# kieranrcampbell/clonealign

Hardware: AMD Instinct MI355X
Metric: ELBO iterations/sec (higher is better)
Workload: dtype f32 variables (contraction: float64 series over gene bins; count-matrix products: int8 MFMA, exact); 1 GPU; synthetic 100000 cells x 5000 genes x 8 clones, K=1, S=1, cell-sharded over 1 GPU(s) (BASELINE.json configs[2]); cells=100000, genes=5000, clones=8, K=1, mc_samples=1, y_storage=u8, y_bytes_per_elem=1, fused_sweep=True, fwd_mfma=True, series_form=True, y_mfma=True, parallelism=single, collective=none, allreduce_doubles_per_train_pass=20764, build_id=212aa564458010f1

## Files before the change

clonealign_amd/csrc/ca_eng_create.inc:

```

constexpr double CA_ML_STREAM_FIXED_US = 6.6;
constexpr double CA_ML_STREAM_BYTES_PER_US = 5.62e6;
constexpr double CA_ML_MIN_STREAM_US = 45.0;
constexpr int CA_ML_MAX_PER = 4;
struct ca_mom_last_in {
  int slots;
  int n_cu;
  int nb_stream, nb_ovf;
  int ngrp, nred;
  int64_t image_bytes;
};
inline int ca_mom_last_free(const ca_mom_last_in& a) { return std::max(a.slots - a.nb_stream, 0); }
inline int ca_mom_last_free_x(const ca_mom_last_in& a) {
  const int xcd = std::max(a.n_cu / 32, 1);
  return a.slots / xcd - cdiv(a.nb_stream, xcd);
}
inline int ca_mom_last_per(const ca_mom_last_in& a) {
  const int xcd = std::max(a.n_cu / 32, 1), free_x = ca_mom_last_free_x(a);
  if (free_x < 1) return 0;
  return std::max(1, cdiv(a.ngrp, free_x * xcd));
}
inline bool ca_mom_last_pick(const ca_mom_last_in& a) {
  if (a.nb_stream + a.ngrp + a.nred <= a.slots) return false;
  const int per = ca_mom_last_per(a);
// ... 413 lines not shown
          HIPCK(h, hipGetLastError());
          int total = 0;
          HIPCK(h, hipMemcpyAsync(&total, h->esc2_off + nkeys, sizeof(int), hipMemcpyDeviceToHost, h->stream));
          SYNC(h);
          if ((int64_t)total != ne) { h->err = "2-bit image: the device's escape count differs from the host plan's"; return CA_ERR_STATE; }
          h->n_esc2 = total;
          CACK(dalloc(h, &h->esc2, h->n_esc2));
          hipLaunchKernelGGL(k_esc_fill, dim3(cdiv(nw * 64, CA_YM_TB)), dim3(CA_YM_TB), 0, h->stream, (const uint8_t*)h->Y, Nn, h->Gp, h->ys_nseg, h->ys_RS,
                             h->esc2_off, h->esc2, (const uint4*)h->y2_pos, n2);
          const int64_t sb = n2 * 1024 + (8 - n2) * 2048, ib = (h->ys_N64 / 64) * h->ys_nseg * sb;
          CACK(dalloc(h, &h->Ys2, ib));
          hipLaunchKernelGGL(k_pack_y2, dim3(cdiv(ib / 16, CA_YM_TB)), dim3(CA_YM_TB), 0, h->stream, (const uint8_t*)h->Y, (uint4*)h->Ys2, Nn, h->ys_N64, h->Gp, n2,
                             h->y2_perm);
          HIPCK(h, hipGetLastError());
          SYNC(h);
          h->ys_n2 = n2;
          h->y_dev_bytes += ib + 4 * h->n_esc2 + 4 * (nkeys + 1) + 4 * (int64_t)h->Gp;
        }
      }
    }
    if (h->adam_bound > 0) h->ys_step_bound = (float)(1.02 * h->adam_bound);
    h->y_ys = true;
    h->y_dev_bytes += h->ys4 ? h->ys_N64 * h->Gp / 2 + 4 * h->n_esc + 4 * ((int64_t)h->ys_nrg * h->ys_nseg * 4 * h->ys_RS + 1) : h->ys_N64 * h->Gp;
  }
  h->mom_ride = h->poly && h->y_ys && !h->poly_side && h->host_dev && variant_on(h, CA_VAR_MOM_RIDE, "CA_MOM_RIDE");
  if (h->mom_ride) {
    ca_mom_last_in ml;
    int per_cu = 0;
    const hipError_t oe = h->ys4 ? (h->n_ovf > 0 ? hipOccupancyMaxActiveBlocksPerMultiprocessor(&per_cu, k_ys_mfma_ovf_mom<true>, CA_YM_TB, CA_YS4_LDS_BYTES)
                                                 : hipOccupancyMaxActiveBlocksPerMultiprocessor(&per_cu, k_ys_mfma_mom<true>, CA_YM_TB, CA_YS4_LDS_BYTES))
                                 : (h->n_ovf > 0 ? hipOccupancyMaxActiveBlocksPerMultiprocessor(&per_cu, k_ys_mfma_ovf_mom<false>, CA_YM_TB, CA_YS_LDS_BYTES)
                                                 : hipOccupancyMaxActiveBlocksPerMultiprocessor(&per_cu, k_ys_mfma_mom<false>, CA_YM_TB, CA_YS_LDS_BYTES));
    if (oe != hipSuccess) { (void)hipGetLastError(); per_cu = 0; }
    ml.slots = per_cu * h->n_cu; ml.n_cu = h->n_cu;
    ml.nb_stream = h->ys_nrg * h->ys_nseg;
    ml.nb_ovf = h->n_ovf > 0 ? cdiv(Nn, CA_TB) + cdiv(h->n_ovf_chunk, CA_TB / 64) : 0;
    ml.ngrp = h->pws.n_gene_blocks; ml.nred = CA_MOM_NRED;
    ml.image_bytes = h->ys_N64 * h->Gp / (h->ys4 ? 2 : 1);
    h->mom_free_slots = ca_mom_last_free(ml);
    h->mom_last = variantx_on(h, CA_VARX_MOM_LAST, "CA_MOM_LAST_ON") || (variant_on(h, CA_VAR_MOM_LAST, "CA_MOM_LAST") && ca_mom_last_pick(ml));
    if (h->opt.variant_off & CA_VAR_MOM_LAST) h->mom_last = false;
    if (h->mom_last) {
      const int per = ca_mom_last_per(ml);
      h->mom_per = per < 1 ? CA_MOM_PER : std::min(per, CA_ML_MAX_PER);
      h->mom_nred = 2 * CA_MOM_NRED;
      const int lab = (h->opt.reserved[1] & ~0xFF) ? h->opt.reserved[1] >> 8 : 0;
      if (lab & 15) h->mom_per = lab & 15;
      if (lab & 16) h->mom_nred = CA_MOM_NRED;
      h->mom_ovf_first = (lab & 32) != 0;
    }
  }
  h->cell_lean = h->poly && variant_on(h, CA_VAR_CELL_LEAN, "CA_CELL_LEAN");
  h->cell_mfma = h->poly && variant_on(h, CA_VAR_CELL_MFMA, "CA_CELL_MFMA");
  h->ride_ok = h->ystore == CA_YSTORE_U8 && K == 1 && D <= 2 && h->fused_ok && !h->c16 && h->fwd_cell && (h->fc_tl == 6 || h->fc_tl == 8 || (h->fc_tl == 2 && h->fc_nbig == 0)) &&
               !h->y_ys && variant_on(h, CA_VAR_Y_RIDE, "CA_Y_RIDE");
  const bool tl1_ok = h->fc_tl == 1 && h->fc_nbig == 0 && !h->c16;
  h->ride_ys = h->y_ys && (!h->ys4 || (h->poly && D == 1 && !h->c16 && !h->s2)) && D <= 2 && h->fused_ok && h->fwd_cell && (h->fc_tl == 6 || tl1_ok || (h->fc_tl == 2 && h->fc_nbig == 0)) &&
               variant_on(h, CA_VAR_Y_RIDE, "CA_Y_RIDE");
  h->yfin_split = h->ride_ys && h->bwd_mfma && h->tail_fuse && variant_on(h, CA_VAR_YFIN_RIDE, "CA_YFIN_RIDE");
  if (h->y_ys && !h->ride_ys) h->async_y = false;
  {
    const int tiles = cdiv(Nn, 16), qb = tiles / std::max(h->n_cu, 1), rb = tiles - qb * h->n_cu;
    h->fwd_bal = h->ride_ys && !h->c16 && !h->s2 && D == 1 && C <= 8 && qb >= 1 && qb <= 6 && h->nk32 >= 96 && h->host_dev && variant_on(h, CA_VAR_FWD_BAL, "CA_FWD_BAL");
    if (h->fwd_bal) {
      h->bal_q = qb; h->bal_r = rb;
      h->bal_nchunk = rb > 0 ? std::min(CA_BAL_MAXCHUNK, h->n_cu / rb) : 0;
      CACK(dalloc(h, &h->bal_xw, std::max<int64_t>(1, (int64_t)rb * h->bal_nchunk * 512)));
    }
  }
  h->s2f = h->s2 && h->fused_ok && h->fwd_cell && (h->fc_tl == 2 || h->fc_tl == 6) && (h->ride_ys || !h->ride_ok) && variant_on(h, CA_VAR_S2_FUSE, "CA_S2_FUSE");
  h->layout_series = h->poly || (h->poly_shape && h->opt.world > 1);
  if (h->layout_series) {
    h->off_y = 3 + C;
    h->off_q = h->off_y + (int64_t)h->Gp * K;
    h->off_x = h->off_q + (int64_t)CA_PL_NB * (CA_PL_R + 2) * 8;
    h->off_g = h->off_x + std::max(h->opt.world, 1);
    h->red_n = h->off_g + (int64_t)G * (S + D);
    CACK(dalloc(h, &h->red, h->red_n));
    if (h->poly) h->pws.tabQ = h->red + h->off_q;
  } else {
  h->off_g = 3 + C;
  h->off_y = h->off_g + (int64_t)G * (S + D);
  h->red_n = h->off_y + (int64_t)G * K;
  CACK(dalloc(h, &h->red, h->off_y + (int64_t)h->Gp * std::max(K, 1)));
  }
  CACK(dalloc(h, &h->terms_dev, 4));
  CACK(ensure_elbo_cap(h, 64));
  CACK(ensure_eps_cap(h, 1));
  {
    const int cols = 1 + ((K > 0) ? P : 0);
    const int cols_all = cols + (p->loc0 ? 0 : 1);
    std::vector<double> srow;
    if (!p->loc0) {
      srow.resize((size_t)Nn);
      HIPCK(h, hipMemcpyAsync(srow.data(), h->s64, (size_t)Nn * sizeof(double), hipMemcpyDeviceToHost, h->stream));
      SYNC(h);
    }
    std::vector<double> cs((size_t)G, 0.0), ytx((size_t)G * std::max(P, 1), 0.0);
    float *Ft = nullptr, *Vt = nullptr, *YWp = nullptr, *YTp = nullptr; double* yt = nullptr;
    HIPCK(h, hipMalloc((void**)&Ft, (size_t)Nn * sizeof(float)));
    HIPCK(h, hipMalloc((void**)&Vt, (size_t)G * sizeof(float)));
    HIPCK(h, hipMalloc((void**)&YWp, (size_t)h->nseg * Nn * sizeof(float)));
    HIPCK(h, hipMalloc((void**)&YTp, (size_t)h->nrb * h->Gp * sizeof(float)));
    HIPCK(h, hipMalloc((void**)&yt, (size_t)h->Gp * sizeof(double)));
    HIPCK(h, hipMemsetAsync(Vt, 0, (size_t)G * sizeof(float), h->stream));
    std::vector<float> col((size_t)Nn);
// ... 63 lines not shown
```

clonealign_amd/csrc/ca_eng_loop.inc:

```
int wait_y(ca_engine* h, bool all) {
  if (all) {
    if (h->y_pending) HIPCK(h, hipStreamWaitEvent(h->stream, h->ev_ydone, 0));
    h->y_pending = false; h->yw_pending = false;
  } else if (h->yw_pending) {
    HIPCK(h, hipStreamWaitEvent(h->stream, h->ev_ywdone, 0));
    h->yw_pending = false;
  }
  return CA_OK;
}

int make_etamax(ca_engine* h) {
  if (h->D > 0) {
    LAUNCH(h, CA_KERNEL_OTHER, hipLaunchKernelGGL(k_vmm_final, dim3(1), dim3(64), 0, h->stream, h->vmm_part, h->vmm, h->ngblk, h->D));
    LAUNCH(h, CA_KERNEL_OTHER, hipLaunchKernelGGL(k_etamax, dim3(cdiv(h->N, CA_TB)), dim3(CA_TB), 0, h->stream, h->F, h->vmm, h->etamax2, h->N, h->D));
  }
  h->em_stale = false;
  return CA_OK;
}
int ensure_etamax(ca_engine* h) {
  if (!h->em_stale) return CA_OK;
  return make_etamax(h);
}

int refresh_derived(ca_engine* h) {
  CACK(wait_y(h, true));
  h->y_defer = false;
  h->pre_valid = false;
  h->ys_steps = -1;
  h->ys_quant_ready = false;
  if (h->D > 0) LAUNCH(h, CA_KERNEL_OTHER, hipLaunchKernelGGL(k_vprep, dim3(h->ngblk), dim3(CA_TB), 0, h->stream, h->V, h->Vs, h->vmm_part, h->G, h->D));
  CACK(make_etamax(h));
  h->gaux_slot = -1;
  h->ycache_valid = false;
  h->yfin_pending = false;
  h->look_valid = false;
  h->poly_fresh = false;
  h->poly_seq_base = h->poly_seq + 1;
  h->poly_xmax_ready = false;
  h->poly_xglob_steps = -1;
  return CA_OK;
}

ca_ovf_args ovf_args(ca_engine* h, float* YWextra) {
  ca_ovf_args ovf;
  memset(&ovf, 0, sizeof(ovf));
  if (h->n_ovf > 0) {
    ovf.nb_rows = cdiv(h->N, CA_TB); ovf.nb_chunks = cdiv(h->n_ovf_chunk, CA_TB / 64);
    ovf.rowptr = h->ovf_rowptr; ovf.col = h->ovf_col; ovf.val = h->ovf_val; ovf.YWextra = YWextra;
    ovf.chunk_start = h->ovf_chunk_start; ovf.row2 = h->ovf_row2; ovf.val2 = h->ovf_val2; ovf.csum = h->ovf_csum; ovf.nchunk = h->n_ovf_chunk;
  }
  return ovf;
}
ca_yfin_args yfin_args(ca_engine* h, int rows, int nseg) {
  ca_yfin_args a;
  memset(&a, 0, sizeof(a));
  a.ncol = cdiv((int64_t)h->Gp * h->K, 64); a.nrow = h->n_yw;
  a.part = h->YTpart; a.out = h->red + h->off_y; a.rows = rows; a.ld = (int64_t)h->Gp * h->K; a.cols = h->Gp * h->K; a.G = h->G;
  if (h->n_ovf > 0) { a.col_chunk_ptr = h->ovf_col_chunk_ptr; a.csum = h->ovf_csum; }
  a.YWpart = h->YWpart; a.nseg = nseg + (h->n_ovf > 0 ? 1 : 0); a.F = h->F; a.D = h->D; a.N = h->N; a.YW = h->YW; a.yw_part = h->yw_part;
  return a;
}
int launch_yfinish(ca_engine* h, int rows, int nseg) {
  const ca_yfin_args a = yfin_args(h, rows, nseg);
  LAUNCH(h, CA_KERNEL_OTHER, hipLaunchKernelGGL(k_yfinish, dim3(a.ncol + a.nrow), dim3(1024), 0, h->stream, a.part, a.out, a.rows, a.ld, a.cols, a.col_chunk_ptr,
                                                a.csum, h->K, a.G, a.ncol, a.YWpart, a.nseg, a.F, a.D, a.N, a.YW, a.yw_part));
  return CA_OK;
}

ca_ysq_args ys_quant_args(ca_engine* h, int steps, bool* lagged) {
  ca_ysq_args a;
  memset(&a, 0, sizeof(a));
  const int s0 = h->ys_slot, s1 = (s0 + 1) % 3;
  a.nblk = h->ys_nq;
  a.V = h->V; a.Dv = h->D; a.G = h->G; a.GS = h->Gp / 64; a.F = h->F; a.Df = h->D; a.N = h->N; a.NS = h->ys_N64 / 64;
  *lagged = steps >= 0 && steps <= 4 && h->ys_step_bound > 0.f;
  if (*lagged) {
    a.amax_in = h->ys_amaxp + (int64_t)s0 * h->ys_ncap * 2; a.n_in = h->ys_namax[s0];
    a.slack_w = a.slack_p = (float)steps * h->ys_step_bound;
  } else {
    a.amax_in = reinterpret_cast<const float*>(h->ys_amax); a.n_in = 1;
  }
  a.amax_out = h->ys_amaxp + (int64_t)s1 * h->ys_ncap * 2;
  h->ys_namax[s1] = h->ys_nq;
  a.exps = h->ys_exps + 2 * s0; a.Wr = h->Wr; a.Pr = h->Pr; a.Wsum = h->Wsum; a.Psum = h->Psum;
  return a;
}
int ys_quant(ca_engine* h) {
  if (h->ys_quant_ready) return CA_OK;
  bool lagged = false;
  ca_ysq_args a = ys_quant_args(h, h->ys_steps, &lagged);
  if (!lagged) {
    HIPCK(h, hipMemsetAsync(h->ys_amax, 0, 2 * sizeof(unsigned), h->stream));
    LAUNCH(h, CA_KERNEL_OTHER, hipLaunchKernelGGL(k_ym_absmax, dim3(cdiv(std::max<int64_t>(h->N, h->G), CA_YM_TB)), dim3(CA_YM_TB), 0, h->stream,
                                                  h->V, h->D, (int64_t)h->G, h->F, h->D, h->N, 1, h->ys_amax));
  }
  LAUNCH(h, CA_KERNEL_OTHER, hipLaunchKernelGGL(k_ys_quant, dim3(a.nblk), dim3(CA_YM_TB), 0, h->stream, a));
  return CA_OK;
}
ca_ys_io ys_io(ca_engine* h) {
  ca_ys_io io;
  io.Wr = h->Wr; io.Pr = h->Pr; io.Wsum = h->Wsum; io.Psum = h->Psum; io.exps = h->ys_exps + 2 * h->ys_slot;
  io.YWpart = h->YWpart; io.YTpart = h->YTpart;
  io.esc_off = h->ys4 ? h->esc_off : nullptr; io.esc = h->ys4 ? h->esc : nullptr;
  io.perm = nullptr;
  return io;
}
ca_ovf_args ys_ovf(ca_engine* h) { return ovf_args(h, h->YWpart + (int64_t)h->ys_nseg * h->N); }
int yfin_flush(ca_engine* h) {
  if (!h->yfin_pending) return CA_OK;
  h->yfin_pending = false;
  return launch_yfinish(h, h->ys_nrg, h->ys_nseg);
}
int ys_finish(ca_engine* h, bool defer = false) {
  h->yfin_pending = true;
  if (!defer) CACK(yfin_flush(h));
  h->ys_slot = (h->ys_slot + 1) % 3;
  h->ys_launched = true;
  h->ys_steps = 0;
  h->ys_quant_ready = false;
  h->ycache_valid = true;
  return CA_OK;
}
template <bool Y4, int N2 = 0>
void launch_ys(ca_engine* h) {
  constexpr int lds = Y4 ? CA_YS4_LDS_BYTES : CA_YS_LDS_BYTES;
  ca_ys_io yio = ys_io(h);
  const uint8_t* Yimg = h->Ys;
  if (N2 > 0) { Yimg = h->Ys2; yio.esc_off = h->esc2_off; yio.esc = h->esc2; yio.perm = h->y2_perm; }
  const int nb_main = h->ys_nrg * h->ys_nseg;
  const ca_pm_args* pm = h->mom_args;
  h->mom_args = nullptr;
  const int nmom = pm ? pm->nmb + pm->nred : 0;
  if (h->n_ovf > 0) {
    const ca_ovf_args ovf = ys_ovf(h);
    const dim3 grid(nmom + nb_main + ovf.nb_rows + ovf.nb_chunks);
    if (pm) {
      ca_pm_args pmo = *pm;
      if (h->mom_last && h->mom_ovf_first) pmo.blk0 += ovf.nb_rows + ovf.nb_chunks;
      hipLaunchKernelGGL((k_ys_mfma_ovf_mom<Y4, N2>), grid, dim3(CA_YM_TB), lds, h->stream, Yimg, yio, h->N, h->Gp, h->ys_RS, nb_main, ovf, h->F, h->V, h->D, pmo);
    }
    else hipLaunchKernelGGL((k_ys_mfma_ovf<Y4, N2>), grid, dim3(CA_YM_TB), lds, h->stream, Yimg, yio, h->N, h->Gp, h->ys_RS, nb_main, ovf, h->F, h->V, h->D);
  } else {
    if (pm) hipLaunchKernelGGL((k_ys_mfma_mom<Y4, N2>), dim3(nmom + nb_main), dim3(CA_YM_TB), lds, h->stream, Yimg, yio, h->N, h->Gp, h->ys_RS, *pm);
    else hipLaunchKernelGGL((k_ys_mfma<Y4, N2>), dim3(nb_main), dim3(CA_YM_TB), lds, h->stream, Yimg, yio, h->N, h->Gp, h->ys_RS);
  }
}
int ycache_ys(ca_engine* h) {
  CACK(ys_quant(h));
  if (h->ys4 && h->ys_n2 == 6) LAUNCH(h, CA_KERNEL_YPASS, (launch_ys<true, 6>(h)));
  else if (h->ys4 && h->ys_n2 == 5) LAUNCH(h, CA_KERNEL_YPASS, (launch_ys<true, 5>(h)));
  else if (h->ys4) LAUNCH(h, CA_KERNEL_YPASS, launch_ys<true>(h));
  else LAUNCH(h, CA_KERNEL_YPASS, launch_ys<false>(h));
  const bool defer = h->ys_defer_next;
  h->ys_defer_next = false;
  return ys_finish(h, defer);
}

int ensure_ycache(ca_engine* h) {
  if (h->y_defer) {
    h->y_defer = false;
    HIPCK(h, hipStreamWaitEvent(h->stream2, h->ev_params, 0));
    std::swap(h->stream, h->stream2);
    h->on_side = true;
    const int rc = ensure_ycache(h);
    h->on_side = false;
    std::swap(h->stream, h->stream2);
    CACK(rc);
    HIPCK(h, hipEventRecord(h->ev_ydone, h->stream2));
    h->y_pending = true;
    HIPCK(h, hipEventRecord(h->ev_ywdone, h->stream2));
    h->yw_pending = true;
    return CA_OK;
  }
  if (h->ycache_valid || h->K == 0) { h->ycache_valid = true; return yfin_flush(h); }
  h->yfin_pending = false;
  if (h->y_ys) return ycache_ys(h);
  dim3 grid((unsigned)((int64_t)h->nrg * h->nseg));
  const ca_ovf_args ovf = ovf_args(h, h->YWpart + (int64_t)h->nseg * h->N * h->K);
  ca_ovf_args none;
  memset(&none, 0, sizeof(none));
  const ca_ypass_ops fit = {h->F, h->D, h->V, h->YWpart, h->YTpart, h->K};
  for (int koff = 0; koff < h->K; koff += 4) {
    const int kk = std::min(4, h->K - koff);
    CACK(prof_begin(h, CA_KERNEL_YPASS));
    const ca_ovf_args& o = koff == 0 ? ovf : none;
    ypass<0>(h, fit, koff, kk, grid, o);
    HIPCK(h, hipGetLastError());
    CACK(prof_end(h));
  }
  if (!h->on_side) {
    CACK(launch_yfinish(h, h->nrg, h->nseg));
  } else {
    LAUNCH(h, CA_KERNEL_OTHER, hipLaunchKernelGGL(k_colsum, dim3(cdiv((int64_t)h->Gp * h->K, 64)), dim3(1024), 0, h->stream,
                                                  h->YTpart, h->red + h->off_y, h->nrg, (int64_t)h->Gp * h->K, h->Gp * h->K,
                                                  h->n_ovf > 0 ? h->ovf_col_chunk_ptr : nullptr, h->n_ovf > 0 ? h->ovf_csum : nullptr, h->K, h->G));
    LAUNCH(h, CA_KERNEL_OTHER, hipLaunchKernelGGL(k_yw_dot, dim3(h->n_yw), dim3(CA_TB), 0, h->stream, h->YWpart,
                                                  h->nseg + (h->n_ovf > 0 ? 1 : 0), h->F, h->D, h->K, h->N, h->YW, h->yw_part));
  }
  h->ycache_valid = true;
  return CA_OK;
}


ca_small_args small_args(ca_engine* h, const double* gene_part, int apply, float lr_t, double* elbo_dst, bool reduce_cells) {
  ca_small_args a;
  a.enabled = 1;
  a.red = h->red; a.gene_part = gene_part; a.ngblk = h->ngblk;
  a.vchi = h->vchi; a.alpha_u = h->alpha_u; a.m_v = h->m_v; a.v_v = h->v_v; a.m_a = h->m_a; a.v_a = h->v_a; a.g_v = h->g_v; a.g_a = h->g_a;
  a.elbo_out = elbo_dst; a.terms_out = h->terms_dev;
  a.G = h->G; a.C = h->C; a.K = h->K; a.apply = apply;
  a.lr_t = lr_t; a.b1 = (float)h->opt.beta1; a.b2 = (float)h->opt.beta2; a.aeps = (float)h->opt.adam_eps;
  a.vmm_part = h->vmm_part; a.vmm = h->vmm; a.D = h->D;
  a.dir_const = h->dir_const;
  a.cell_part = reduce_cells ? h->cell_part : nullptr; a.ncblk = h->ncblk;
  a.host_out = nullptr; a.host_flag = nullptr; a.host_seq = 0; a.reduce_only = 0;
  a.yw_part = nullptr; a.n_yw = 0;
  a.ee_part = nullptr; a.n_ee = 0;
  a.vchi_out = nullptr; a.alpha_out = nullptr;
  if (!apply && elbo_dst && h->host_seq_next && h->host_dev) {
    a.host_out = h->host_dev + 32;
    a.host_flag = reinterpret_cast<unsigned long long*>(h->host_dev + 33);
    a.host_seq = h->host_seq_next;
    h->host_seq_next = 0;
  }
  return a;
}
int mon_tail_local_sums(ca_engine* h) {
  if (!h->mon_tail.enabled || !h->mon_tail.cell_part) return CA_OK;
  CACK(wait_y(h, false));
  ca_small_args r = h->mon_tail;
  r.reduce_only = 1; r.host_out = nullptr;
  LAUNCH(h, CA_KERNEL_OTHER, hipLaunchKernelGGL(k_final_small, dim3(1), dim3(CA_TB), 0, h->stream, r));
  h->mon_tail.cell_part = nullptr; h->mon_tail.yw_part = nullptr;
  return CA_OK;
}
int flush_mon_tail(ca_engine* h) {
  if (!h->mon_tail.enabled) return CA_OK;
  CACK(wait_y(h, false));
  if (h->mon_tail.yw_part) CACK(yfin_flush(h));
  if (is_sharded(h) && (h->mon_tail.cell_part || h->mon_tail_local)) {
    CACK(mon_tail_local_sums(h));
    CACK(allreduce(h, h->red, 3 + h->C));
    h->mon_tail_local = false;
  }
  LAUNCH(h, CA_KERNEL_OTHER, hipLaunchKernelGGL(k_final_small, dim3(1), dim3(CA_TB), 0, h->stream, h->mon_tail));
  h->mon_tail.enabled = 0;
  return CA_OK;
}

#ifndef CA_BWD_TL3_MAXN
#define CA_BWD_TL3_MAXN 18432
#endif
int train_bwd(ca_engine* h, const float* mu32, bool cell_sums_global) {
  const int W_ = h->S + h->D;
  bool merged = false, ride_ar = false;
  ca_ar_ride ride;
  if (h->poly_fresh) {
    h->poly_fresh = false;
    h->fold_now = false;
    CACK(yfin_flush(h));
    ca_small_args bwd_tail = no_small_args();
    if (is_sharded(h)) {
      bool local_sums = false;
      if (h->mon_tail.enabled && h->mon_tail.cell_part) { CACK(mon_tail_local_sums(h)); local_sums = true; }
      else if (h->mon_tail.enabled && h->mon_tail_local) local_sums = true;
      h->mon_tail_local = false;
      CACK(wait_y(h, true));
      if (!h->poly_xslot_pending)
        HIPCK(h, ca_poly_xslot(h->stream, h->poly_xmax_ready ? h->poly_xpart : nullptr, (int)cdiv(h->N, CA_TB), h->F, h->N, h->red + h->off_x, h->opt.rank,
                               std::max(h->opt.world, 1)));
      h->poly_xslot_pending = false;
      const int64_t skip = (cell_sums_global && !local_sums) ? 3 + h->C : 0;
      CACK(allreduce(h, h->red + skip, h->off_g - skip));
      h->poly_xglob_steps = 0;
      CACK(prof_begin(h, CA_KERNEL_BWD));
      const hipError_t e = ca_poly_backward(h->stream, &h->pws, h->V, mu32, h->Lb, h->G, h->C, h->red + h->off_g, nullptr);
      HIPCK(h, e);
      CACK(prof_end(h));
      h->poly_df = true;
      h->ycache_valid = false;
      return CA_OK;
    }
    else if (h->mon_tail.enabled && h->mon_tail.cell_part && h->upd_merge && h->opt.reserved[1] != 6) {
      CACK(wait_y(h, false));
      bwd_tail = h->mon_tail;
      bwd_tail.reduce_only = 1; bwd_tail.host_out = nullptr;
      h->mon_tail.cell_part = nullptr; h->mon_tail.yw_part = nullptr;
    }
    else if (h->mon_tail.enabled) { CACK(wait_y(h, false)); bwd_tail = h->mon_tail; h->mon_tail.enabled = 0; }
    CACK(prof_begin(h, CA_KERNEL_BWD));
    const hipError_t e = ca_poly_backward(h->stream, &h->pws, h->V, mu32, h->Lb, h->G, h->C, h->red + h->off_g, &bwd_tail);
    HIPCK(h, e);
    CACK(prof_end(h));
    h->poly_df = true;
  } else
  if (h->bwd_mfma) {
    h->poly_df = false;
    const int xb = cdiv(h->nwt, CA_TB / 64);
    ca_yfin_args yfin;
    memset(&yfin, 0, sizeof(yfin));
    ride_ar = is_sharded(h) && p2p_ride_ok(h, h->red_n);
    if (is_sharded(h) && !ride_ar) CACK(yfin_flush(h));
    if (h->yfin_pending) { yfin = yfin_args(h, h->ys_nrg, h->ys_nseg); h->yfin_pending = false; }
    ca_small_args bwd_tail = no_small_args();
    bool split_tail = false;
    if (h->mon_tail.enabled && h->mon_tail.cell_part) {
      CACK(wait_y(h, false));
      bwd_tail = h->mon_tail;
      merged = is_sharded(h);
      if (merged) { bwd_tail.reduce_only = 1; bwd_tail.host_out = nullptr; }
      if (merged && ride_ar && yfin.nrow > 0 && bwd_tail.yw_part) {
        ride.yw_part = bwd_tail.yw_part; ride.n_yw = bwd_tail.n_yw; ride.yw_index = 0;
        bwd_tail.yw_part = nullptr;
      }
      split_tail = !merged && yfin.nrow > 0 && bwd_tail.yw_part != nullptr;
      if (split_tail) { bwd_tail.reduce_only = 1; bwd_tail.host_out = nullptr; bwd_tail.yw_part = nullptr; }
    }
    const int nextra = (bwd_tail.enabled || yfin.nrow) ? 1 + cdiv(yfin.ncol, CA_TB / 64) + yfin.nrow : 0;
    const ca_bwdm_extra extra = {bwd_tail, yfin, cdiv(nextra, xb)};
    const bool s2b = h->s2f && h->S == 2 && !h->c16;
    ca_bwdm_ops o;
    memset(&o, 0, sizeof(o));
    if (h->bwd_pairs) {
      for (int s = 0; s < h->S; ++s)
        for (int pr = 0; pr < h->bwd_pairs; ++pr) {
          const bool lone = (h->nchunk & 1) && pr == h->bwd_pairs - 1;
          o.coefq = h->coefq + ((int64_t)s * h->bwd_pairs + pr) * h->N16 * 32; o.Lb = h->Lb + (int64_t)pr * 2 * h->G * CA_CW; o.mu = mu32 + (int64_t)s * h->G;
          o.sidx = s; o.first_s = pr == 0 ? 1 : 0; o.extra = (s == 0 && pr == 0) ? &extra : nullptr;
          o.c16 = !lone;
          o.coefq1 = lone ? nullptr : h->coefq + ((int64_t)(h->S + s) * h->bwd_pairs + pr) * h->N16 * 32;
          CACK(launch_bwd_mfma(h, h->D == 1 ? 1 : 2, o));
        }
    } else {
      o.Lb = h->Lb; o.first_s = 1; o.frac = h->bwd_frac; o.c16 = h->c16; o.s2 = s2b; o.tl3 = h->bwd_tl == 3;
      if ((h->D == 1 || h->D == 2) && (s2b || h->c16)) o.coefq1 = h->coefq + h->N16 * 32;
      if ((h->D == 1 || h->D == 2) && s2b) o.mu1 = mu32 + h->G;
      for (int s = 0; s < (s2b ? 1 : h->S); ++s) {
        o.coefq = h->coefq + (int64_t)s * h->N16 * 32; o.mu = mu32 + (int64_t)s * h->G; o.sidx = s; o.extra = s == 0 ? &extra : nullptr;
        CACK(launch_bwd_mfma(h, h->D, o));
      }
    }
    if (bwd_tail.enabled) {
      if (merged) { h->mon_tail.cell_part = nullptr; h->mon_tail.yw_part = nullptr; }
      else if (split_tail) h->mon_tail.cell_part = nullptr;
      else h->mon_tail.enabled = 0;
    }
    h->fold_now = h->fold_gsum && !is_sharded(h);
    if (ride_ar) { ride.gpart = h->gpart; ride.nslice = h->csplit_m; ride.fold_n = (int64_t)h->G * W_; }
    else if (!h->fold_now)
      LAUNCH(h, CA_KERNEL_OTHER,
             hipLaunchKernelGGL(k_colsum, dim3(cdiv((int64_t)h->G * W_, 64)), dim3(1024), 0, h->stream, h->gpart,
                                h->red + h->off_g, h->csplit_m, (int64_t)h->G * W_, h->G * W_));
  } else {
    h->fold_now = false;
// ... 20 lines not shown
  CACK(wait_y(h, true));
  if (h->poly && is_sharded(h)) {
    HIPCK(h, ca_poly_xslot(h->stream, h->poly_xmax_ready ? h->poly_xpart : nullptr, (int)cdiv(h->N, CA_TB), h->F, h->N, h->red + h->off_x, h->opt.rank,
                           std::max(h->opt.world, 1)));
    h->poly_xglob_steps = 0;
    h->poly_xslot_pending = false;
  }
  const int64_t skip = (cell_sums_global && !merged) ? 3 + h->C : 0;
  ride.fold_lo = h->off_g - skip;
  CACK(allreduce(h, h->red + skip, h->red_n - skip, ride_ar ? &ride : nullptr));
  if (is_sharded(h)) h->ycache_valid = false;
  return CA_OK;
}

inline bool update_merges(const ca_engine* h, int apply, const double* elbo_dst) {
  const int64_t mB = h->s2 ? 2 * h->hint_A + 1 : h->hint_B;
  return apply && h->upd_merge && !elbo_dst && h->pre_ok && h->hint_A >= 0 && mB >= 0 && h->fused_ok && h->gene_part_alt && h->fwd_cell && h->K > 0;
}
ca_pre_args pre_args(const ca_engine* h, int64_t A, int64_t B) {
  ca_pre_args pre;
  memset(&pre, 0, sizeof(pre));
  pre.nblk = h->ngblk;
  pre.loc = h->loc; pre.ls = h->ls; pre.epsA = h->eps_dev + A * (int64_t)h->G; pre.epsB = h->eps_dev + B * (int64_t)h->G;
  pre.colsum = h->colsum; pre.Lb = h->Lb; pre.V = h->V; pre.YtX = h->YtX; pre.muA = h->mu32; pre.muB = h->s2 ? h->mu32 + h->G : h->mu32B; pre.Mb = h->Mb2;
  pre.s2 = h->s2 ? 1 : 0;
  pre.gene_partA = h->gene_part_alt; pre.gene_partB = h->gene_partB_alt; pre.Mq = h->fwd_mfma ? h->Mq : nullptr;
  pre.G = h->G; pre.D = h->D; pre.K = h->K; pre.mrow = h->frow; pre.C = h->C;
  return pre;
}
ca_ysq_args ys_quant_ride(ca_engine* h) {
  ca_ysq_args a;
  memset(&a, 0, sizeof(a));
  if (!h->y_ys || h->K == 0 || h->ys_quant_ready) return a;
  bool lagged = false;
  const ca_ysq_args q = ys_quant_args(h, h->ys_steps >= 0 ? h->ys_steps + 1 : -1, &lagged);
  if (!lagged) return a;
  h->ys_quant_ready = true;
  return q;
}
int defer_y_to_side(ca_engine* h) {
  if (!h->async_y || h->K == 0 || h->ride_ok || h->ride_ys) return CA_OK;
  HIPCK(h, hipEventRecord(h->ev_params, h->stream));
  h->y_defer = true;
  return CA_OK;
}
void adam_stepped(ca_engine* h, bool xmax_ready) {
  if (h->ys_steps >= 0) h->ys_steps += 1;
  h->b1p *= (float)h->opt.beta1;
  h->b2p *= (float)h->opt.beta2;
  h->adam_steps += 1;
  h->poly_xmax_ready = xmax_ready;
  if (h->poly_xglob_steps >= 0) h->poly_xglob_steps += 1;
  h->ycache_valid = false;
  h->yfin_pending = false;
  h->look_valid = false;
  if (h->poly && h->y_ys && h->K > 0) h->poly_y_defer = true;
}
int train_update(ca_engine* h, const float* eps, int apply, double* elbo_dst) {
  const int N256 = cdiv(h->N, CA_TB);
  float lr_t = 0.f;
  if (apply) {
    lr_t = (float)h->opt.learning_rate * sqrtf(1.f - h->b2p) / (1.f - h->b1p);
  }
  CACK(yfin_flush(h));
  ca_small_args mon = no_small_args();
  if (h->mon_tail.enabled) { mon = h->mon_tail; h->mon_tail.enabled = 0; }
  ca_psi_args psi;
  memset(&psi, 0, sizeof(psi));
  if (h->K > 0) {
    psi.nblk = N256; psi.F = h->F; psi.YW = h->YW; psi.dFpart = h->dFpart; psi.m_psi = h->m_psi; psi.v_psi = h->v_psi; psi.g_psi = h->g_psi;
    psi.N = h->N; psi.D = h->D; psi.K = h->K; psi.ntile = h->poly_df ? 1 : h->bwd_mfma ? cdiv(h->nwt, CA_TB / 64) : h->ntile;
  }
  h->pre_valid = false;
  {
    int64_t mA = h->hint_A, mB = h->hint_B;
    if (h->s2) { mA = 2 * h->hint_A; mB = mA + 1; }
    if (update_merges(h, apply, elbo_dst)) {
      ca_merge_args mg;
      memset(&mg, 0, sizeof(mg));
      h->gate_armed = false;
      if (h->gate_req && h->host_dev) {
        mg.gate = reinterpret_cast<const unsigned long long*>(h->host_dev + 48); mg.gate_seq = ++h->gate_seq;
        mg.gate_ack = reinterpret_cast<unsigned long long*>(h->host_dev + 56);
        mg.gate_err = reinterpret_cast<unsigned long long*>(h->host_dev + 40);
        mg.gate_local = h->gate_local;
        mg.gate_timeout = h->gate_ticks;
        h->gate_armed = true;
        h->gate_t0 = std::chrono::steady_clock::now();
      }
      h->gate_req = false;
      mg.pre = pre_args(h, mA, mB);
      mg.ysq = ys_quant_ride(h);
      if (mg.ysq.nblk) {
        mg.ysq.nblk = h->ngblk + N256;
        h->ys_namax[(h->ys_slot + 1) % 3] = h->ngblk + N256;
      }
      mg.tail = small_args(h, h->gene_part, 1, lr_t, nullptr, false);
      mg.tail.terms_out = nullptr;
      mg.tail.vmm_part = nullptr; mg.tail.vmm = nullptr;
      mg.tail.vchi_out = h->vchi_alt; mg.tail.alpha_out = h->alpha_u_alt;
      mg.glogit = h->glogit; mg.dgl = h->dgl; mg.m_gl = h->m_gl; mg.v_gl = h->v_gl; mg.C = h->C; mg.ncell = N256;
      if (!h->vmm_at_ready) {
        int init[32];
        for (int i = 0; i < 32; ++i) init[i] = (i & 8) ? (int)0x807FFFFF  : (int)0x7F800000 ;
        HIPCK(h, hipMemcpyAsync(h->vmm_at, init, sizeof(init), hipMemcpyHostToDevice, h->stream));
        HIPCK(h, hipStreamSynchronize(h->stream));
        h->vmm_at_ready = true;
// ... 116 lines not shown
      const hipError_t q = hipStreamQuery(h->stream);
      if (q != hipSuccess && q != hipErrorNotReady) HIPCK(h, q);
      if ((q == hipSuccess && e[0] != (double)want) || std::chrono::steady_clock::now() >= t_end) {
        h->err = "internal: the ranges of an earlier pass never reached the host (series form's look ahead)";
        return CA_ERR_STATE;
      }
    }
  }
  std::atomic_thread_fence(std::memory_order_acquire);
  out[0] = e[1]; out[1] = e[2]; out[2] = e[3];
  return CA_OK;
}
struct ca_xsrc { const float* xpart; int nx; const double* xglob; int nglob; double xadd; };
inline double poly_step_bound(const ca_engine* h) {
  return h->adam_bound * 1.0001;
}
int poly_xsrc(ca_engine* h, ca_xsrc* x) {
  memset(x, 0, sizeof(*x));
  const int nx = (int)cdiv(h->N, CA_TB);
  if (is_sharded(h)) {
    const int W = std::max(h->opt.world, 1);
    if (h->poly_xglob_steps < 0 || h->poly_xglob_steps > 1) {
      HIPCK(h, ca_poly_xslot(h->stream, h->poly_xmax_ready ? h->poly_xpart : nullptr, nx, h->F, h->N, h->red + h->off_x, h->opt.rank, W));
      CACK(allreduce(h, h->red + h->off_x, W));
      h->poly_xglob_steps = 0;
      h->poly_xslot_pending = false;
    }
    x->xglob = h->red + h->off_x; x->nglob = W; x->xadd = (double)h->poly_xglob_steps * poly_step_bound(h);
  } else if (h->poly_xmax_ready) { x->xpart = h->poly_xpart; x->nx = nx; }
  return CA_OK;
}
int poly_guard(ca_engine* h, bool* use_series, double** mirror, double* seq, bool* ranges_queued) {
  const uint64_t s = h->poly_seq + 1;
  *ranges_queued = false;
  *mirror = h->poly_ring_dev + (s % 16) * 4;
  *seq = (double)s;
  double r[3];
  int steps;
  if (s < h->poly_seq_base + CA_POLY_LAG) {
    if (s == h->poly_seq_base) {
      ca_xsrc xs;
      CACK(poly_xsrc(h, &xs));
      HIPCK(h, ca_poly_ranges(h->stream, &h->pws, h->V, h->F, h->G, h->N, *mirror, *seq, xs.xpart, xs.nx, xs.xglob, xs.nglob, xs.xadd));
      *ranges_queued = true;
      h->poly_steps_at[s % 16] = h->adam_steps;
    }
    CACK(poly_wait_entry(h, h->poly_seq_base, r));
    steps = (int)(h->adam_steps - h->poly_steps_at[h->poly_seq_base % 16]);
  } else {
    CACK(poly_wait_entry(h, s - CA_POLY_LAG, r));
    steps = (int)(h->adam_steps - h->poly_steps_at[(s - CA_POLY_LAG) % 16]);
  }
  *use_series = ca_poly_covers(r[0], r[1], r[2], steps, poly_step_bound(h));
  h->poly_seq = s;
  h->poly_steps_at[s % 16] = h->adam_steps;
  return CA_OK;
}

int fused_pass(ca_engine* h, int64_t slotA, int64_t slotB, double* elbo_dst, double* elbo_dstB = nullptr, int64_t trainA = -1) {
  const bool s2f = trainA >= 0;
  const float* epsA = h->eps_dev + slotA * (int64_t)h->G;
  const float* epsB = h->eps_dev + slotB * (int64_t)h->G;
  if (elbo_dstB) CACK(flush_mon_tail(h));
  if (h->pre_valid && h->pre_A == slotA && h->pre_B == slotB) {
    std::swap(h->gene_part, h->gene_part_alt);
    std::swap(h->gene_partB, h->gene_partB_alt);
  } else {
    LAUNCH(h, CA_KERNEL_OTHER,
           hipLaunchKernelGGL(k_gene_pre_fused, dim3(h->ngblk), dim3(CA_TB), 0, h->stream, h->loc, h->ls, epsA, epsB, h->colsum, h->Lb,
                              h->V, h->D, h->K, h->YtX, h->mu32, h->s2 ? h->mu32 + h->G : h->mu32B, h->Mb2, h->gene_part, h->gene_partB, h->G,
                              h->frow, h->C, h->fwd_mfma ? h->Mq : nullptr, h->s2 ? 1 : 0));
  }
  if (s2f) {
    const float* epsTA = h->eps_dev + trainA * (int64_t)h->G;
    LAUNCH(h, CA_KERNEL_OTHER,
           hipLaunchKernelGGL(k_gene_pre_fused, dim3(h->ngblk), dim3(CA_TB), 0, h->stream, h->loc, h->ls, epsTA, epsTA + h->G, h->colsum, h->Lb,
                              h->V, h->D, h->K, h->YtX, h->mu32, h->mu32 + h->G, h->Mb2, h->gene_partB, h->gene_partB, h->G,
                              h->frow, h->C, h->Mq + (int64_t)h->nk32 * 1024, 1));
  }
  h->pre_valid = false;
  h->poly_fresh = false;
  bool series = h->poly && !s2f && !elbo_dstB && !h->fwd_gate && (!is_sharded(h) || h->opt.world <= CA_TB);
  double* pl_mirror = nullptr; double pl_seq = 0.0;
  if (series) {
    bool queued = false;
    CACK(poly_guard(h, &series, &pl_mirror, &pl_seq, &queued));
    if (!series && !queued) {
      ca_xsrc xs;
      CACK(poly_xsrc(h, &xs));
      HIPCK(h, ca_poly_ranges(h->stream, &h->pws, h->V, h->F, h->G, h->N, pl_mirror, pl_seq, xs.xpart, xs.nx, xs.xglob, xs.nglob, xs.xadd));
    }
    if (series) h->n_series += 1; else h->n_series_fallback += 1;
  }
  const bool ride = (h->ride_ok || h->ride_ys) && !h->ycache_valid && h->fwd_cell && !h->y_defer && !h->y_pending && !series;
  if (!ride && !series) CACK(ensure_ycache(h));
  ca_cell_ptrs cp;
  cp.A = h->A; cp.cn = h->cn; cp.s64 = h->s64; cp.etamax2 = h->etamax2; cp.glogit = h->glogit; cp.F = h->F;
  cp.coef = h->coef; cp.dgl = h->dgl; cp.coefq = h->bwd_mfma ? h->coefq : nullptr;
  cp.vmm_at = nullptr; cp.etamax_w = nullptr;
  cp.gate = nullptr; cp.gate_go = 0ull;
  if (h->fwd_gate) {
    if (!(h->fwd_cell && ride && h->ride_ys) || !h->gate_local) { h->err = "internal: a forward sweep queued ahead of the host's decision must be the one-launch form"; return CA_ERR_STATE; }
    cp.gate = h->gate_local; cp.gate_go = (h->gate_seq << 1) | 1ull;
  }
  if (series) {}
  else if (h->em_stale && h->fwd_cell && h->D > 0) { cp.vmm_at = h->vmm_at + 16 * (1 - h->vmm_at_idx); cp.etamax_w = h->etamax2; h->em_stale = false; }
// ... 5 lines not shown
    cp.etamax2 = h->poly_zero; cp.coefq = nullptr; cp.vmm_at = nullptr; cp.etamax_w = nullptr;
    ca_xsrc xs_m;
    CACK(poly_xsrc(h, &xs_m));
    const bool moments_aside = h->opt.reserved[1] == 4 && h->stream3 && h->ev_poly0 && !h->ycache_valid && !h->poly_side && !h->y_pending;
    if (moments_aside) {
      HIPCK(h, hipEventRecord(h->ev_poly0, h->stream));
      HIPCK(h, hipStreamWaitEvent(h->stream3, h->ev_poly0, 0));
      std::swap(h->stream, h->stream3);
    }
    hipError_t e = hipSuccess;
    ca_pm_args pm;
    const bool mom_rides = h->mom_ride && h->y_ys && !h->ycache_valid && !h->poly_side && !moments_aside && !h->y_defer && !h->y_pending && h->host_dev &&
                           ((xs_m.xpart && xs_m.nx > 0) || (xs_m.xglob && xs_m.nglob > 0));
    if (mom_rides) {
      memset(&pm, 0, sizeof(pm));
      const int nglob = xs_m.xglob ? xs_m.nglob : 0;
      pm.V = h->V; pm.xbits = h->pws.xbits; pm.muA = h->mu32; pm.muB = h->mu32B; pm.Lb = h->Lb; pm.G = h->G; pm.C = h->C;
      pm.hdr = h->pws.hdr; pm.part = h->pws.partB; pm.bad_word = reinterpret_cast<unsigned int*>(h->host_dev + 42); pm.mirror = pl_mirror; pm.seq = pl_seq;
      pm.xpart = xs_m.xpart; pm.nx = (nglob || !xs_m.xpart) ? 0 : xs_m.nx; pm.xglob = xs_m.xglob; pm.nglob = nglob; pm.xadd = xs_m.xadd;
      pm.tabB = h->pws.tabB; pm.flags = h->pws.mflags;
      if (++h->mom_tag == 0u) h->mom_tag = 1u;
      pm.tag = h->mom_tag;
      pm.ngrp = h->pws.n_gene_blocks; pm.per = h->mom_per; pm.nmb = (int)cdiv(pm.ngrp, pm.per); pm.nred = h->mom_nred;
      pm.blk0 = h->mom_last ? h->ys_nrg * h->ys_nseg : 0;
      pm.timeout_ticks = 50000000ull;
      pm.err = reinterpret_cast<unsigned int*>(h->host_dev + 43);
      h->mom_args = &pm;
    } else {
      CACK(prof_begin(h, CA_KERNEL_FWD));
      e = ca_poly_moments(h->stream, &h->pws, h->V, h->F, h->mu32, h->mu32B, h->Lb, h->G, h->N, h->C,
                          h->host_dev ? reinterpret_cast<unsigned int*>(h->host_dev + 42) : nullptr, pl_mirror, pl_seq,
                          xs_m.xpart, xs_m.nx, xs_m.xglob, xs_m.nglob, xs_m.xadd);
      int pe = (e == hipSuccess) ? prof_end(h) : CA_OK;
      if (moments_aside) {
        if (e == hipSuccess) e = hipEventRecord(h->ev_poly1, h->stream);
        std::swap(h->stream, h->stream3);
      }
      HIPCK(h, e);
      CACK(pe);
    }
    if (h->poly_side && h->poly_y_defer && !h->ycache_valid) {
      h->poly_y_defer = false;
      HIPCK(h, hipEventRecord(h->ev_params, h->stream));
      h->y_defer = true;
    }
    h->ys_defer_next = h->y_ys && !h->ycache_valid && h->opt.reserved[1] != 3;
    const int yrc = ensure_ycache(h);
    const bool mom_left = h->mom_args != nullptr;
    h->mom_args = nullptr;
    CACK(yrc);
    if (mom_left) { h->err = "internal: the series form's moments were to ride on a count-matrix stream launch that was not made"; return CA_ERR_STATE; }
    h->ys_defer_next = false;
    ca_yfin_args yfin_ride;
    const bool yfin_rides = h->yfin_pending;
    if (yfin_rides) { yfin_ride = yfin_args(h, h->ys_nrg, h->ys_nseg); h->yfin_pending = false; }
    if (moments_aside) HIPCK(h, hipStreamWaitEvent(h->stream, h->ev_poly1, 0));
    CACK(prof_begin(h, CA_KERNEL_FWD));
    ca_small_args ltail = no_small_args();
    const bool sh = is_sharded(h) && h->tail_fuse && yfin_rides;
    if (sh) {
      ltail = small_args(h, h->gene_part, 0, 0.f, nullptr, true);
      ltail.ncblk = h->pws.n_cell_blocks;
      if (h->K > 0) { ltail.yw_part = h->yw_part; ltail.n_yw = h->n_yw; }
      ltail.reduce_only = 1; ltail.host_out = nullptr;
    }
    e = ca_poly_cells(h->stream, &h->pws, h->N, h->C, h->K, &cp, h->alpha_u, h->cell_part, h->dFpart, yfin_rides ? &yfin_ride : nullptr,
                      sh ? &ltail : nullptr, h->poly_xmax_ready ? h->poly_xpart : nullptr, (int)cdiv(h->N, CA_TB), h->F, sh ? h->red + h->off_x : nullptr,
                      h->opt.rank, std::max(h->opt.world, 1), h->cell_lean, h->cell_mfma);
    h->mon_tail_local = sh;
    if (sh) { h->poly_xslot_pending = true; h->poly_xglob_steps = -1; }
    HIPCK(h, e);
    CACK(prof_end(h));
    cell_blocks = h->pws.n_cell_blocks;
    h->poly_fresh = true;
  } else
  if (h->fwd_cell && ride && h->ride_ys) {
    cell_blocks = h->ncblk_f;
    CACK(ys_quant(h));
    ca_ysride_args ya;
    memset(&ya, 0, sizeof(ya));
    ya.Ys = h->Ys; ya.io = ys_io(h); ya.F = h->F; ya.V = h->V; ya.Df = h->D;
    ya.Gp = h->Gp; ya.RS = h->ys_RS; ya.nb_main = h->ys_nrg * h->ys_nseg; ya.nb_y = ya.nb_main;
    ya.ovf = ys_ovf(h);
    ya.nb_y += ya.ovf.nb_rows + ya.ovf.nb_chunks;
    if (h->fwd_bal && !s2f) {
      ca_bal_args ba;
      memset(&ba, 0, sizeof(ba));
      ba.nb = h->n_cu; ba.r = h->bal_r; ba.nchunk = h->bal_nchunk; ba.xw = h->bal_xw;
      cell_blocks = h->n_cu;
      if (++h->bal_tag == 0u) h->bal_tag = 1u;
      ba.tag = h->bal_tag;
      ba.timeout_ticks = 50000000ull;
      ba.err = reinterpret_cast<unsigned int*>(h->host_dev + 41);
      ba.stream_units = h->opt.ride_pattern == 2 ? 2 : 1;
      CACK(launch_fwd_bal_ys(h, cp, ba, ya));
    } else CACK(launch_fwd_cell_mix_ys(h, cp, ya, s2f));
    CACK(ys_finish(h, h->yfin_split && (!is_sharded(h) || p2p_ride_ok(h, h->red_n))));
  } else if (h->fwd_cell && ride) {
    cell_blocks = h->ncblk_f;
    ca_yride_args ya;
    memset(&ya, 0, sizeof(ya));
    ya.Y = (const uint8_t*)h->Y; ya.F = h->F; ya.Dstride = h->D; ya.V = h->V; ya.YWpart = h->YWpart; ya.YTpart = h->YTpart;
    ya.G = h->G; ya.Gp = h->Gp; ya.nseg = h->nseg; ya.nrb = h->nrb; ya.TR = h->TR;
    ya.nb_main = h->nrg * h->nseg; ya.nb_y = ya.nb_main;
    ya.ovf = ovf_args(h, h->YWpart + (int64_t)h->nseg * h->N * h->K);
    ya.nb_y += ya.ovf.nb_rows + ya.ovf.nb_chunks;
    CACK(launch_fwd_cell_mix_y(h, cp, ya));
    CACK(launch_yfinish(h, h->nrg, h->nseg));
    h->ycache_valid = true;
  } else if (h->fwd_cell) {
    cell_blocks = h->ncblk_f;
    CACK(launch_fwd_cell(h, cp, s2f));
  } else {
  if (h->fwd_mfma) {
    CACK(launch_fwd_mfma(h, h->Mq, h->Zpart2, h->fsplit, h->fkchunk));
  } else {
    LAUNCH(h, CA_KERNEL_FWD, launch_fwd_fused(h->C, h->D, dim3(cdiv(h->N, CA_TB * kFwdR), h->gsplit), h->stream, h->F, h->etamax2,
                                              h->Vs, h->Mb2, h->Zpart2, h->N, h->G, h->gchunk));
  }
  {
    CACK(launch_cell_fused(h, cp));
// ... 158 lines not shown
```

clonealign_amd/csrc/ca_eng_reduce.inc:

```
inline bool is_sharded(const ca_engine* h) { return h->opt.world > 1 || h->comm || h->host_ar || (h->p2p && h->p2p->connected); }
struct ca_ar_ride {
  const float* gpart = nullptr; int nslice = 0; int64_t fold_lo = 0, fold_n = 0;
  const double* yw_part = nullptr; int n_yw = 0; int64_t yw_index = -1;
};
inline bool p2p_ride_ok(const ca_engine* h, int64_t n) { return h->p2p && h->p2p->connected && h->p2p_ride && n <= h->p2p->cap; }
int allreduce(ca_engine* h, double* buf, int64_t n, const ca_ar_ride* ride = nullptr) {
  if (h->opt.world <= 1 && !h->comm && !h->host_ar && !(h->p2p && h->p2p->connected)) return CA_OK;
  if (h->p2p && h->p2p->connected) {
    ca_p2p* pp = h->p2p;
    for (int64_t o = 0; o < n; o += pp->cap) {
      const int64_t m = std::min<int64_t>(pp->cap, n - o);
      const int nblk = (int)std::max<int64_t>(1, std::min<int64_t>(cdiv(m, CA_TB), 64));
      ca_p2p_args a;
      memset(&a, 0, sizeof(a));
      a.peers = pp->peers_dev; a.rank = h->opt.rank; a.world = h->opt.world; a.cap = pp->cap;
      a.seq = ++pp->seq; a.err = pp->err_dev; a.err_local = pp->err_local; a.timeout_ticks = pp->timeout_ticks;
      a.yw_index = -1;
      if (ride) {
        a.gpart = ride->gpart; a.nslice = ride->nslice; a.fold_lo = ride->fold_lo; a.fold_n = ride->fold_n;
        a.yw_part = ride->yw_part; a.n_yw = ride->n_yw; a.yw_index = ride->yw_index;
      }
      LAUNCH(h, CA_KERNEL_OTHER, hipLaunchKernelGGL(k_p2p_allreduce, dim3(nblk), dim3(CA_TB), 0, h->stream, buf + o, m, a));
    }
    return CA_OK;
  }
  if (h->host_ar) {
    if (n > h->host_ar_cap) {
      if (h->host_ar_buf) HIPCK(h, hipHostFree(h->host_ar_buf));
      HIPCK(h, hipHostMalloc((void**)&h->host_ar_buf, (size_t)n * sizeof(double)));
      h->host_ar_cap = n;
    }
    HIPCK(h, hipMemcpyAsync(h->host_ar_buf, buf, (size_t)n * sizeof(double), hipMemcpyDeviceToHost, h->stream));
    SYNC(h);
    if (h->host_ar(h->host_ar_user, h->host_ar_buf, n) != 0) { h->err = "host all-reduce callback failed"; return CA_ERR_COMM; }
    HIPCK(h, hipMemcpyAsync(buf, h->host_ar_buf, (size_t)n * sizeof(double), hipMemcpyHostToDevice, h->stream));
    return CA_OK;
  }
  if (!h->comm) { h->err = "world > 1 but neither ca_comm_init() nor ca_set_host_allreduce() was called"; return CA_ERR_STATE; }
  int rc = g_rccl.AllReduce(buf, buf, (size_t)n, kNcclFloat64, kNcclSum, h->comm, h->stream);
  if (rc != 0) {
    h->err = std::string("ncclAllReduce: ") + (g_rccl.GetErrorString ? g_rccl.GetErrorString(rc) : "error");
    return CA_ERR_COMM;
  }
  return CA_OK;
}
```

clonealign_amd/csrc/ca_eng_state.inc:

```
namespace {

thread_local std::string g_last_error;

typedef struct { char internal[128]; } ca_nccl_uid;
typedef void* ca_nccl_comm;
struct RcclApi {
  void* lib = nullptr;
  int (*GetUniqueId)(ca_nccl_uid*) = nullptr;
  int (*CommInitRank)(ca_nccl_comm*, int, ca_nccl_uid, int) = nullptr;
  int (*CommDestroy)(ca_nccl_comm) = nullptr;
  int (*AllReduce)(const void*, void*, size_t, int, int, ca_nccl_comm, hipStream_t) = nullptr;
  const char* (*GetErrorString)(int) = nullptr;
  std::string err;
  bool load() {
    if (lib) return true;
    const char* cands[] = {getenv("CLONEALIGN_RCCL_LIB"), "librccl.so.1", "librccl.so", "/opt/rocm/lib/librccl.so.1",
                           "/opt/rocm/lib/librccl.so"};
    for (const char* c : cands) {
      if (!c || !*c) continue;
      lib = dlopen(c, RTLD_NOW | RTLD_LOCAL);
      if (lib) break;
    }
    if (!lib) { err = std::string("cannot dlopen librccl: ") + dlerror(); return false; }
    GetUniqueId = (decltype(GetUniqueId))dlsym(lib, "ncclGetUniqueId");
    CommInitRank = (decltype(CommInitRank))dlsym(lib, "ncclCommInitRank");
    CommDestroy = (decltype(CommDestroy))dlsym(lib, "ncclCommDestroy");
    AllReduce = (decltype(AllReduce))dlsym(lib, "ncclAllReduce");
    GetErrorString = (decltype(GetErrorString))dlsym(lib, "ncclGetErrorString");
    if (!GetUniqueId || !CommInitRank || !CommDestroy || !AllReduce) { err = "librccl lacks expected symbols"; return false; }
    return true;
  }
};
RcclApi g_rccl;
constexpr int kNcclFloat64 = 8;
constexpr int kNcclSum = 0;

struct EvPair { hipEvent_t a, b; int kid; };

}

struct ca_p2p {
  double* slab = nullptr; size_t slab_bytes = 0; int64_t cap = 0;
  std::vector<void*> opened;
  double** peers_dev = nullptr;
  unsigned long long seq = 0;
  bool mapped = false;
  bool connected = false;
  unsigned long long* err_host = nullptr;
  unsigned long long* err_dev = nullptr;
  unsigned int* err_local = nullptr;
  unsigned long long timeout_ticks = 0;
};
struct ca_p2p_wire {
  hipIpcMemHandle_t mem; int64_t cap; int32_t rank, world, device, pid;
  uint64_t local_ptr;
};
static_assert(sizeof(ca_p2p_wire) <= CA_P2P_HANDLE_BYTES, "handle too small");

inline double ca_adam_step_bound(double lr, double b1, double b2) {
  if (!(b1 >= 0 && b2 > 0 && b1 * b1 < b2 && b2 < 1 && lr > 0)) return -1.0;
  double sup = 0.0, p1 = 1.0, p2 = 1.0;
  for (int t = 1; t <= 200000; ++t) { p1 *= b1; p2 *= b2; sup = std::max(sup, std::sqrt(1.0 - p2) / (1.0 - p1)); }
  return lr * sup * (1.0 - b1) / std::sqrt((1.0 - b2) * (1.0 - b1 * b1 / b2));
}
struct ca_engine {
  int64_t N = 0;
  int G = 0, C = 0, K = 0, P = 0, S = 0, D = 0;
  int layout = 0;
  int nchunk = 0;
  ca_options opt{};
  int device = 0;
  hipStream_t stream = nullptr;
  hipStream_t stream2 = nullptr; hipEvent_t ev_params = nullptr, ev_ydone = nullptr; bool y_pending = false, async_y = true;
  hipStream_t stream3 = nullptr;
  hipEvent_t ev_poly0 = nullptr, ev_poly1 = nullptr;
  bool poly_xmax_ready = false; float* poly_xpart = nullptr;
  bool ys_defer_next = false;
  std::string err;
  std::vector<void*> allocs;
  int64_t dev_bytes = 0;
  int ystore = 0, ybytes = 0, VEC = 0, Gp = 0, nseg = 0, TR = 0, nrb = 0, nrg = 0;
  void* Y = nullptr;
  int64_t y_dev_bytes = 0;
  int64_t n_ovf = 0;
  int64_t *ovf_rowptr = nullptr, *ovf_chunk_start = nullptr; int* ovf_col_chunk_ptr = nullptr; float* ovf_csum = nullptr; int n_ovf_chunk = 0;
  int *ovf_col = nullptr, *ovf_row2 = nullptr;
  float *ovf_val = nullptr, *ovf_val2 = nullptr;
  std::vector<int> h_orow, h_ocol; std::vector<float> h_oval;
  const ca_sparse* sp_in = nullptr;
  float* Lb = nullptr;
  double *A = nullptr, *cn = nullptr, *s64 = nullptr, *colsum = nullptr, *YtX = nullptr;
  float* s32 = nullptr;
  float *F = nullptr, *m_psi = nullptr, *v_psi = nullptr;
  float *glogit = nullptr, *m_gl = nullptr, *v_gl = nullptr;
  float *V = nullptr, *m_V = nullptr, *v_V = nullptr;
  float *loc = nullptr, *ls = nullptr, *m_loc = nullptr, *v_loc = nullptr, *m_ls = nullptr, *v_ls = nullptr;
  float* loc_init = nullptr;
  float *vchi = nullptr, *m_v = nullptr, *v_v = nullptr;
  float *alpha_u = nullptr, *m_a = nullptr, *v_a = nullptr;
  float *vchi_alt = nullptr, *alpha_u_alt = nullptr;
  bool upd_merge = false, em_stale = false;
  bool run_gate = false, gate_req = false, gate_armed = false;
  unsigned long long gate_ticks = 100000ull; std::chrono::steady_clock::time_point gate_t0;
  double ticks_per_us = 100.0;
  bool gate_open = false, gate_aborted = false, in_run = false; struct gate_snapshot* gate_snap = nullptr; struct fwd_snapshot* gate_fsnap = nullptr;
  bool run_fwd = false;
  bool fwd_gate = false;
  unsigned long long gate_seq = 0; unsigned long long* gate_local = nullptr;
  bool p2p_ride = false;
  double* gaux = nullptr; int64_t gaux_slot = -1;
  int gaux_idx = 0;
  int* vmm_at = nullptr; int vmm_at_idx = 0; bool vmm_at_ready = false;
  double dir_const = 0.0;
  float b1p = 0.f, b2p = 0.f;
  float *g_loc = nullptr, *g_ls = nullptr, *g_V = nullptr, *g_v = nullptr, *g_a = nullptr, *g_psi = nullptr, *dgl = nullptr;
  float* eps_dev = nullptr; int64_t eps_cap = 0;
  float *mu32 = nullptr, *Mb = nullptr, *Vs = nullptr, *vmm = nullptr, *vmm_part = nullptr, *etamax2 = nullptr;
  double* gene_part = nullptr; int ngblk = 0;
  float *Zpart = nullptr, *coef = nullptr; double* scratch = nullptr;
  double* cell_part = nullptr; int ncblk = 0;
  float *gpart = nullptr, *dFpart = nullptr; int gsplit = 1, gchunk = 0, csplit = 1; int64_t cchunk = 0; int RG = 4, ntile = 0;
  float *YWpart = nullptr, *YTpart = nullptr, *YW = nullptr; double* ytpsi = nullptr;
  double* red = nullptr; int64_t red_n = 0, off_g = 0, off_y = 0;
  int64_t off_q = 0, off_x = 0;
  bool poly_shape = false, layout_series = false;
  bool mon_tail_local = false;
  bool poly_xslot_pending = false;
  int poly_xglob_steps = -1;
  double* elbo_dev = nullptr; int64_t elbo_cap = 0; double* terms_dev = nullptr;
  double* host_pinned = nullptr;
  bool ycache_valid = false, sums_global = false, sums_started = false;
  std::vector<double> mu_part;
  bool fused_ok = false, look_valid = false; int64_t look_slot = 0; int frow = 8;
  bool carry = false, carry_builtin = false; std::vector<float> carry_eps;
  int64_t n_series = 0, n_series_fallback = 0;
  double *poly_ring = nullptr, *poly_ring_dev = nullptr; uint64_t poly_seq = 0, poly_seq_base = 1, adam_steps = 0, poly_steps_at[16] = {};
  bool mom_ride = false; unsigned mom_tag = 0; const ca_pm_args* mom_args = nullptr;
  bool mom_last = false, mom_ovf_first = false; int mom_free_slots = 0, mom_per = CA_MOM_PER, mom_nred = CA_MOM_NRED;
  bool cell_mfma = false;
  bool cell_lean = false;
  bool poly = false, poly_side = false, poly_y_defer = false, poly_fresh = false, poly_df = false ; ca_poly_ws pws; float* poly_zero = nullptr; unsigned char* poly_mem = nullptr;
  float *Mb2 = nullptr, *mu32B = nullptr, *Zpart2 = nullptr; double* gene_partB = nullptr;
  bool y_defer = false;
  bool ride_ok = false;
  bool ride_ys = false;
  bool fold_gsum = false, fold_now = false;
  int64_t hint_A = -1, hint_B = -1, pre_A = -1, pre_B = -1;
  bool pre_valid = false, pre_ok = true, pair_elbo = true;
  double* ee_partB = nullptr;
  double *gene_part_alt = nullptr, *gene_partB_alt = nullptr;
  bool bwd_ready = false; int64_t bwd_slot = -1;
  double* yw_part = nullptr; int n_yw = 0;
  bool yfin_split = false, yfin_pending = false;
  ca_small_args mon_tail;
  bool tail_fuse = true;
  double* host_dev = nullptr;
  unsigned long long host_seq = 0, host_seq_next = 0;
  float* eps_stage = nullptr; size_t eps_stage_bytes = 0;
  hipEvent_t ev_stage = nullptr;
  bool fwd_cell = false; int ncblk_f = 0, fc_tl = 4;
  int fc_nbig = 0;
  bool fwd_mfma = false; int fsplit = 1, fkchunk = 1, nk32 = 1; unsigned short* Mq = nullptr;
  bool fwd_bal = false; int bal_q = 0, bal_r = 0, bal_nchunk = 0; unsigned long long* bal_xw = nullptr; unsigned bal_tag = 0;
  bool pfwd = false; int pf_npair = 0, pf_fsplit = 1, pf_kchunk = 1; unsigned short* pf_Mq = nullptr; float* pf_Z = nullptr;
  int bwd_pairs = 0;
  bool bwd_mfma = false, bwd_frac = false, c16 = false, s2 = false, s2f = false;
  unsigned short* coefq = nullptr; int64_t N16 = 0, cchunk_m = 0; int csplit_m = 1, nwt = 0;
  int bwd_tl = CA_BWD_TL;
  uint64_t draw = 0;
  hipEvent_t ev_ywdone = nullptr; bool yw_pending = false, on_side = false;
  bool y_ys = false, ys4 = false; int* esc_off = nullptr; unsigned* esc = nullptr; int64_t n_esc = 0;
  int ys_n2 = 0; uint8_t* Ys2 = nullptr; unsigned short *y2_perm = nullptr, *y2_pos = nullptr; int* esc2_off = nullptr; unsigned* esc2 = nullptr; int64_t n_esc2 = 0;
  uint8_t* Ys = nullptr; uint4 *Wr = nullptr, *Pr = nullptr; int *Wsum = nullptr, *Psum = nullptr;
  int* ys_exps = nullptr;
  unsigned* ys_amax = nullptr;
  float* ys_amaxp = nullptr; int ys_nq = 0;
  int ys_ncap = 0, ys_namax[3] = {0, 0, 0};
  bool ys_launched = false;
  bool ys_quant_ready = false;
  int ys_slot = 0, ys_steps = -1, ys_RS = 256, ys_nrg = 0, ys_nseg = 0; int64_t ys_N64 = 0; float ys_step_bound = -1.f;
  double adam_bound = -1.0;
  ca_p2p* p2p = nullptr;
  ca_nccl_comm comm = nullptr;
  ca_host_allreduce_fn host_ar = nullptr; void* host_ar_user = nullptr; double* host_ar_buf = nullptr; int64_t host_ar_cap = 0;
  std::vector<EvPair> ev_pool; size_t ev_used = 0; bool prof_open = false;
  unsigned prof_seen[CA_KERNEL_COUNT] = {0, 0, 0, 0, 0};
  double k_ms[CA_KERNEL_COUNT] = {0}; int64_t k_n[CA_KERNEL_COUNT] = {0};
  int n_cu = 256;
};

namespace {

#define HIPCK(h, call)                                                                       \
  do {                                                                                       \
    hipError_t e_ = (call);                                                                  \
    if (e_ != hipSuccess) {                                                                  \
      (h)->err = std::string(#call) + ": " + hipGetErrorString(e_);                          \
      return CA_ERR_HIP;                                                                     \
    }                                                                                        \
  } while (0)

#define CACK(call)                \
  do {                            \
    int rc_ = (call);             \
    if (rc_ != CA_OK) return rc_; \
  } while (0)

int comm_check(ca_engine* h) {
  if (h->host_pinned && *reinterpret_cast<volatile unsigned int*>(h->host_pinned + 41) != 0u) {
    h->err = "a forward-sweep block gave up waiting for a chunk of a left-over tile (k_fwd_bal_ys); the engine's state is undefined";
    return CA_ERR_STATE;
  }
  if (h->host_pinned && *reinterpret_cast<volatile unsigned int*>(h->host_pinned + 43) != 0u) {
    h->err = "a reducer block of the series form's moment role gave up waiting for the moment blocks of its launch (k_ys_mfma_mom); the engine's state is undefined";
    return CA_ERR_STATE;
  }
  if (h->host_pinned && *reinterpret_cast<volatile unsigned int*>(h->host_pinned + 42) != 0u) {
    h->err = "the series form of the contraction (CA_VARX_SERIES) cannot cover this fit's exponent range: max|psi| (max W - min W) exceeds 4 x " +
             std::to_string(CA_PL_NB) + " bins' worth; the passes since are truncated -- start over without the series form";
    return CA_ERR_STATE;
  }
  if (h->p2p && h->p2p->err_host && *reinterpret_cast<volatile unsigned long long*>(h->p2p->err_host) != 0ull) {
    h->err = "peer-to-peer all-reduce #" + std::to_string(*reinterpret_cast<volatile unsigned long long*>(h->p2p->err_host)) +
             ": a peer's data did not arrive within the time limit (peer lost or out of step); this engine's transport is dead -- "
             "destroy the engine and start over in a fresh process";
    return CA_ERR_COMM;
  }
  return CA_OK;
}
#define SYNC(h)                                          \
  do {                                                   \
    HIPCK(h, hipStreamSynchronize((h)->stream));         \
    CACK(comm_check(h));                                 \
  } while (0)

template <typename T>
int dalloc(ca_engine* h, T** p, int64_t n) {
  if (n <= 0) n = 1;
  void* q = nullptr;
  hipError_t e = hipMalloc(&q, (size_t)n * sizeof(T));
  if (e != hipSuccess) {
    h->err = std::string("hipMalloc of ") + std::to_string(n * sizeof(T)) + " bytes: " + hipGetErrorString(e);
    return CA_ERR_NOMEM;
  }
  e = hipMemsetAsync(q, 0, (size_t)n * sizeof(T), h->stream);
  if (e == hipSuccess) e = hipStreamSynchronize(h->stream);
  if (e != hipSuccess) { h->err = hipGetErrorString(e); return CA_ERR_HIP; }
  h->allocs.push_back(q);
  h->dev_bytes += n * (int64_t)sizeof(T);
  *p = (T*)q;
  return CA_OK;
}

struct ca_call_mem {
  hipStream_t stream;
  std::string* err;
  int oom;
  std::vector<void*> owned;
  int rc = CA_OK;
  ca_call_mem(hipStream_t stream_, std::string* err_, int oom_ = CA_ERR_HIP) : stream(stream_), err(err_), oom(oom_) {}
  explicit ca_call_mem(ca_engine* h) : ca_call_mem(h->stream, &h->err) {}
  ca_call_mem(const ca_call_mem&) = delete;
  ca_call_mem& operator=(const ca_call_mem&) = delete;
  ~ca_call_mem() { release(); }
  void release() {
    if (!owned.empty()) hipStreamSynchronize(stream);
    for (void* p : owned) hipFree(p);
    owned.clear();
  }
// ... 253 lines not shown
```

clonealign_amd/csrc/ca_poly.h:

```cpp
#pragma once
#include <hip/hip_runtime.h>
#include <stddef.h>
#include <stdint.h>

#define CA_PL_R 20
#define CA_PL_NB 32
#define CA_PL_A 2.0
#ifndef CA_PL_NBL
#define CA_PL_NBL 4
#endif

struct ca_poly_hdr { double vlo, delta, xmax; int nb, bad; };
struct ca_poly_ws {
  ca_poly_hdr* hdr; unsigned int* xbits; unsigned int* mflags ; double *tabB, *partB, *tabQ, *Qpart;
  int n_cell_blocks, n_gene_blocks;
};

inline bool ca_poly_ok(int D, int S, int C) { return D == 1 && S == 1 && C >= 3 && C <= 8; }
size_t ca_poly_workspace_bytes(int G, int n_cell_blocks);
void ca_poly_bind(ca_poly_ws* w, void* base, int G, int n_cell_blocks);
hipError_t ca_poly_moments(hipStream_t st, const ca_poly_ws* w, const float* V, const float* F, const float* muA, const float* muB, const float* Lb, int G,
                           int64_t N, int C, unsigned int* bad_word ,
                           double* mirror , double seq, const float* xpart, int nx,
                           const double* xglob , int nglob, double xadd);
hipError_t ca_poly_ranges(hipStream_t st, const ca_poly_ws* w, const float* V, const float* F, int G, int64_t N, double* mirror, double seq, const float* xpart, int nx,
                          const double* xglob, int nglob, double xadd);
hipError_t ca_poly_xslot(hipStream_t st, const float* xpart, int nx, const float* F, int64_t N, double* slots, int rank, int world);
inline bool ca_poly_covers(double xmax, double vlo, double vhi, int steps, double step_bound) {
  const double x = xmax + steps * step_bound, wdt = (vhi - vlo) + 2.0 * steps * step_bound;
  return x == x && wdt == wdt && x * wdt <= 2.0 * CA_PL_A * CA_PL_NB;
}
hipError_t ca_poly_cells(hipStream_t st, const ca_poly_ws* w, int64_t N, int C, int K, const void* cell_ptrs, const float* alpha_u, double* cell_part, float* dF,
                         const void* yfin_args ,
                         const void* local_tail ,
                         const float* xs_part, int xs_n, const float* xs_F, double* xs_slots ,
                         int rank, int world,
                         bool lean ,
                         bool mfma );
hipError_t ca_poly_backward(hipStream_t st, const ca_poly_ws* w, const float* V, const float* mu, const float* Lb, int G, int C, double* red_g,
                            const void* small_tail );
```

clonealign_amd/csrc/ca_poly.hip:

```cpp
#include <hip/hip_runtime.h>
#include <stdint.h>

#include <algorithm>
#include <cstring>
#include <type_traits>

#include "ca_poly.h"

namespace ca_series {
#include "ca_kernels.hip.h"

constexpr int R = CA_PL_R, NB = CA_PL_NB;
#include "ca_polymom.hip.h"
constexpr int TB_B = 384;
constexpr int GPB = CA_PM_GPB;

__device__ __forceinline__ float warp_max(float v) {
#pragma unroll
  for (int o = 32; o > 0; o >>= 1) v = fmaxf(v, __shfl_xor(v, o, 64));
  return v;
}
__device__ __forceinline__ float warp_min(float v) {
#pragma unroll
  for (int o = 32; o > 0; o >>= 1) v = fminf(v, __shfl_xor(v, o, 64));
// ... 221 lines not shown
        double a = mine[(b * RQ + qk) * C + qc];
        for (int s = 0; s < CPB; ++s) a += s_cf[s][qc] * s_xp[s][qk] * s_eb[s][b];
        mine[(b * RQ + qk) * C + qc] = a;
      }
    }
    CA_LAB_CELL_PH_AFTER(qa[0], blockIdx.x, pass, 5);
    __syncthreads();
    CA_LAB_CELL_PH(blockIdx.x, pass, 6);
  }
  ca_cell_fused_finish<CP>(acc, sm, cell_part, blockIdx.x, C);
  if constexpr (MFMA) {
    constexpr int QW = RQ * NBR * CP;
    static_assert(CPB * NB >= QW && CPB * XS >= QW && NBL * (R + 1) * 16 >= QW, "a wave's tiles fit each of the three arrays");
    double* const p1 = &s_eb[0][0], * const p2 = &s_xp[0][0], * const p3 = &s_tb[0][0];
    double* const pw = wv == 1 ? p1 : (wv == 2 ? p2 : p3);
#pragma unroll
    for (int i = 0; i < 2; ++i)
#pragma unroll
      for (int j = 0; j < NCT; ++j)
#pragma unroll
        for (int r = 0; r < 4; ++r) {
          const int k = 16 * i + 4 * r + mk;
          if (wv > 0 && k < RQ) pw[k * (NBR * CP) + j * 16 + mrow] = qm[i][j][r];
        }
    __syncthreads();
    if (wv == 0) {
#pragma unroll
      for (int i = 0; i < 2; ++i)
#pragma unroll
        for (int j = 0; j < NCT; ++j)
#pragma unroll
          for (int r = 0; r < 4; ++r) {
            const int k = 16 * i + 4 * r + mk, col = j * 16 + mrow, b = j * BPT + mbl;
            if (k < RQ && b < nb && mcl < C) mine[(b * RQ + k) * C + mcl] = ((qm[i][j][r] + p1[k * (NBR * CP) + col]) + p2[k * (NBR * CP) + col]) + p3[k * (NBR * CP) + col];
          }
    }
  } else if (qown) {
#pragma unroll
    for (int b = 0; b < NBR; ++b) if (b < nb) mine[(b * RQ + qk) * C + qc] = qa[b];
  }
}

struct ca_xslot_args { const float* xpart; int nx; const float* F; int64_t N; double* slots; int rank, world; };
__device__ __forceinline__ void ca_poly_xslot_body(const ca_xslot_args& a) {
  __shared__ float sx[CA_TB / 64];
  float ax = 0.f;
  if (a.nx > 0) { for (int i = threadIdx.x; i < a.nx; i += CA_TB) ax = fmaxf(ax, a.xpart[i]); }
  else { for (int64_t i = threadIdx.x; i < a.N; i += CA_TB) { const float v = fabsf(a.F[i]); ax = fmaxf(ax, v == v ? v : INFINITY); } }
  ax = warp_max(ax);
  if ((threadIdx.x & 63) == 0) sx[threadIdx.x >> 6] = ax;
  __syncthreads();
  if ((int)threadIdx.x < a.world) a.slots[threadIdx.x] = (int)threadIdx.x == a.rank ? (double)fmaxf(fmaxf(sx[0], sx[1]), fmaxf(sx[2], sx[3])) : 0.0;
}
__global__ void __launch_bounds__(CA_TB) k_poly_red(const double* __restrict__ part, int nblk, int64_t stride, const ca_poly_hdr* __restrict__ hdr, int per_bin,
                                                    int mode, int C, double* __restrict__ out, unsigned int* __restrict__ xbits, int nred, ca_small_args tail,
                                                    ca_xslot_args xs) {
  if ((int)blockIdx.x >= nred) {
    const int e = (int)blockIdx.x - nred;
    if (e == 0 && tail.enabled) ca_final_small_body(tail);
    else if (xs.slots) ca_poly_xslot_body(xs);
    return;
  }
  if (xbits && blockIdx.x == 0 && threadIdx.x == 0) *xbits = 0u;
  ca_pm_red_body<false>(part, nblk, stride, hdr->nb * per_bin, mode, C, out, blockIdx.x * (CA_TB / 64) + (threadIdx.x >> 6), nred * (CA_TB / 64));
}

__global__ void __launch_bounds__(CA_TB) k_poly_gene(const ca_poly_hdr* __restrict__ hdr, const double* __restrict__ tabQ, const float* __restrict__ V,
                                                     const float* __restrict__ mu, const float* __restrict__ Lb, int G, int C,
                                                     double* __restrict__ red_g , ca_small_args tail, int ngblk) {
  constexpr int RQ = R + 2;
  if ((int)blockIdx.x >= ngblk) {
    if (tail.enabled) ca_final_small_body(tail);
    return;
  }
  constexpr int NBL = CA_PL_NBL;
  __shared__ double s_tq[NBL][RQ * 8];
  const int nb = hdr->nb;
  const double vlo = hdr->vlo, delta = hdr->delta;
  for (int i = threadIdx.x; i < (nb < NBL ? nb : NBL) * RQ * C; i += CA_TB) s_tq[i / (RQ * C)][i % (RQ * C)] = tabQ[i];
  __syncthreads();
  const int g = blockIdx.x * CA_TB + threadIdx.x;
  if (g >= G) return;
  const double v = (double)V[g];
  int b = (int)floor((v - vlo) / delta);
  b = b < 0 ? 0 : (b >= nb ? nb - 1 : b);
  const double dv = v - (vlo + ((double)b + 0.5) * delta);
  float lrow[8];
  {
    const float4 l0 = *reinterpret_cast<const float4*>(Lb + (int64_t)g * CA_CW), l1 = *reinterpret_cast<const float4*>(Lb + (int64_t)g * CA_CW + 4);
    lrow[0] = l0.x; lrow[1] = l0.y; lrow[2] = l0.z; lrow[3] = l0.w; lrow[4] = l1.x; lrow[5] = l1.y; lrow[6] = l1.z; lrow[7] = l1.w;
  }
  double s0 = 0.0, s1 = 0.0;
#define CA_PL_GENE(TQ)                                                            \
  _Pragma("unroll")                                                               \
  for (int c = 0; c < 8; ++c) {                                                   \
    if (c < C) {                                                                  \
      double tn = (TQ)[(R + 1) * C + c], tk = (TQ)[R * C + c];                    \
      double q = tk, dq = (double)(R + 1) * tn;                                   \
      _Pragma("unroll 10")                                                        \
      for (int k = R - 1; k >= 0; --k) {                                          \
        tn = tk; tk = (TQ)[k * C + c];                                            \
        q = q * dv + tk;                                                          \
        dq = dq * dv + (double)(k + 1) * tn;                                      \
      }                                                                           \
      const double l = (double)lrow[c];                                           \
      s0 += l * q; s1 += l * dq;                                                  \
    }                                                                             \
  }
  if (nb <= NBL) { CA_PL_GENE(s_tq[b]) }
  else { const double* tq = tabQ + (int64_t)b * RQ * C; CA_PL_GENE(tq) }
#undef CA_PL_GENE
  red_g[(int64_t)g * 2 + 0] = s0;
  red_g[(int64_t)g * 2 + 1] = (double)mu[g] * s1;
}

inline int cdiv_i(int64_t a, int64_t b) { return (int)((a + b - 1) / b); }

}
using namespace ca_series;

size_t ca_poly_workspace_bytes(int G, int n_cell_blocks) {
  const size_t nbg = (size_t)cdiv_i(G, GPB);
  return sizeof(ca_poly_hdr) + 64 + ((nbg * sizeof(unsigned int) + 63) / 64) * 64 + sizeof(double) * ((size_t)NB * (R + 1) * 16 * (nbg + 1) + (size_t)NB * (R + 2) * 8 * ((size_t)n_cell_blocks + 1));
}

void ca_poly_bind(ca_poly_ws* w, void* base, int G, int n_cell_blocks) {
  char* q = static_cast<char*>(base);
  w->hdr = reinterpret_cast<ca_poly_hdr*>(q); q += sizeof(ca_poly_hdr);
  w->xbits = reinterpret_cast<unsigned int*>(q); q += 64;
  const size_t nbg = (size_t)cdiv_i(G, GPB);
  w->mflags = reinterpret_cast<unsigned int*>(q); q += ((nbg * sizeof(unsigned int) + 63) / 64) * 64;
  w->tabB = reinterpret_cast<double*>(q); q += sizeof(double) * (size_t)NB * (R + 1) * 16;
  w->partB = reinterpret_cast<double*>(q); q += sizeof(double) * (size_t)NB * (R + 1) * 16 * nbg;
  w->tabQ = reinterpret_cast<double*>(q); q += sizeof(double) * (size_t)NB * (R + 2) * 8;
  w->Qpart = reinterpret_cast<double*>(q);
  w->n_cell_blocks = n_cell_blocks; w->n_gene_blocks = (int)nbg;
}

__global__ void __launch_bounds__(CA_TB) k_poly_xslot(const float* __restrict__ xpart, int nx, const float* __restrict__ F, int64_t N, double* __restrict__ slots, int rank,
                                                      int world) {
  const ca_xslot_args a = {xpart, nx, F, N, slots, rank, world};
  ca_poly_xslot_body(a);
}
hipError_t ca_poly_xslot(hipStream_t st, const float* xpart, int nx, const float* F, int64_t N, double* slots, int rank, int world) {
  hipLaunchKernelGGL(k_poly_xslot, dim3(1), dim3(CA_TB), 0, st, xpart, xpart ? nx : 0, F, N, slots, rank, world);
  return hipGetLastError();
}

hipError_t ca_poly_ranges(hipStream_t st, const ca_poly_ws* w, const float* V, const float* F, int G, int64_t N, double* mirror, double seq, const float* xpart, int nx,
                          const double* xglob, int nglob, double xadd) {
  if (!xpart) nx = 0;
  if (!xglob) nglob = 0;
  if (nx == 0 && nglob == 0) hipLaunchKernelGGL(k_poly_xmax, dim3((unsigned)std::min<int64_t>(128, (N + 4 * CA_TB - 1) / (4 * CA_TB))), dim3(CA_TB), 0, st, F, N, w->xbits);
  hipLaunchKernelGGL(k_poly_ranges, dim3(1), dim3(CA_TB), 0, st, V, G, w->xbits, mirror, seq, xpart, nglob ? 0 : nx, xglob, nglob, xadd);
  return hipGetLastError();
}

hipError_t ca_poly_moments(hipStream_t st, const ca_poly_ws* w, const float* V, const float* F, const float* muA, const float* muB, const float* Lb, int G,
                           int64_t N, int C, unsigned int* bad_word, double* mirror, double seq, const float* xpart, int nx, const double* xglob, int nglob, double xadd) {
  if (!xpart) nx = 0;
  if (!xglob) nglob = 0;
  if (nx == 0 && nglob == 0) hipLaunchKernelGGL(k_poly_xmax, dim3((unsigned)std::min<int64_t>(128, (N + 4 * CA_TB - 1) / (4 * CA_TB))), dim3(CA_TB), 0, st, F, N, w->xbits);
  ca_pm_args a;
  memset(&a, 0, sizeof(a));
  a.V = V; a.xbits = w->xbits; a.muA = muA; a.muB = muB; a.Lb = Lb; a.G = G; a.C = C; a.hdr = w->hdr; a.part = w->partB; a.bad_word = bad_word; a.mirror = mirror; a.seq = seq;
  a.xpart = xpart; a.nx = nglob ? 0 : nx; a.xglob = xglob; a.nglob = nglob; a.xadd = xadd;
  hipLaunchKernelGGL(k_poly_B, dim3(w->n_gene_blocks), dim3(TB_B), 0, st, a);
  {
    ca_small_args no_tail; memset(&no_tail, 0, sizeof(no_tail));
    ca_xslot_args no_xs; memset(&no_xs, 0, sizeof(no_xs));
    hipLaunchKernelGGL(k_poly_red, dim3(256), dim3(CA_TB), 0, st, w->partB, w->n_gene_blocks, (int64_t)NB * (R + 1) * 16, w->hdr,
                       (R + 1) * 16, 0, C, w->tabB, w->xbits, 256, no_tail, no_xs);
  }
  return hipGetLastError();
}

hipError_t ca_poly_cells(hipStream_t st, const ca_poly_ws* w, int64_t N, int C, int K, const void* cell_ptrs, const float* alpha_u, double* cell_part, float* dF,
                         const void* yfin_args, const void* local_tail, const float* xs_part, int xs_n, const float* xs_F, double* xs_slots, int rank, int world, bool lean, bool mfma) {
  const ca_cell_ptrs& p = *static_cast<const ca_cell_ptrs*>(cell_ptrs);
  ca_yfin_args yfin;
  if (yfin_args) memcpy(&yfin, yfin_args, sizeof(yfin)); else memset(&yfin, 0, sizeof(yfin));
  int CP = 1;
  while (CP < C) CP <<= 1;
  const int nextra = yfin_args ? cdiv_i(yfin.ncol, CA_TB / 64) + yfin.nrow : 0;
  const dim3 grid(w->n_cell_blocks + nextra);
#define CA_PCELL(CPV, LV) do { if (mfma) CA_PCELL_(CPV, LV, true); else CA_PCELL_(CPV, LV, false); } while (0)
#define CA_PCELL_(CPV, LV, MV) hipLaunchKernelGGL((k_poly_cell<CPV, LV, MV>), grid, dim3(CA_TB), 0, st, w->hdr, w->tabB, p, alpha_u, cell_part, N, C, K, dF, w->Qpart, \
                                         w->n_cell_blocks, yfin)
  if (lean) {
    if (K > 1) return hipErrorInvalidValue;
    if (CP == 4) CA_PCELL(4, true); else CA_PCELL(8, true);
  } else {
    if (CP == 4) CA_PCELL(4, false); else CA_PCELL(8, false);
  }
#undef CA_PCELL
#undef CA_PCELL_
  {
    ca_small_args tail;
    if (local_tail) memcpy(&tail, local_tail, sizeof(tail)); else memset(&tail, 0, sizeof(tail));
    const ca_xslot_args xs = {xs_part, xs_part ? xs_n : 0, xs_F, N, xs_slots, rank, world};
    const int nextra = (tail.enabled || xs_slots) ? 2 : 0;
    hipLaunchKernelGGL(k_poly_red, dim3(256 + nextra), dim3(CA_TB), 0, st, w->Qpart, w->n_cell_blocks, (int64_t)NB * (R + 2) * 8, w->hdr,
                       (R + 2) * C, 1, C, w->tabQ, nullptr, 256, tail, xs);
  }
  return hipGetLastError();
}

hipError_t ca_poly_backward(hipStream_t st, const ca_poly_ws* w, const float* V, const float* mu, const float* Lb, int G, int C, double* red_g, const void* small_tail) {
  ca_small_args tail;
  static_assert(sizeof(ca_small_args) <= 512, "ca_small_args");
  if (small_tail) memcpy(&tail, small_tail, sizeof(tail)); else memset(&tail, 0, sizeof(tail));
  const int ngblk = cdiv_i(G, CA_TB);
  hipLaunchKernelGGL(k_poly_gene, dim3(ngblk + (tail.enabled ? 1 : 0)), dim3(CA_TB), 0, st, w->hdr, w->tabQ, V, mu, Lb, G, C, red_g, tail, ngblk);
  return hipGetLastError();
}

#ifdef CA_LAB
extern "C" int ca_lab_read_cell_stamps(unsigned long long* out, int n_words) {
  return hipMemcpyFromSymbol(out, HIP_SYMBOL(ca_series::ca_lab_stamps4), (size_t)n_words * sizeof(unsigned long long)) == hipSuccess ? 0 : 2;
}
#endif
```

clonealign_amd/csrc/ca_polymom.hip.h:

```cpp
#pragma once
#include "ca_poly.h"

#ifndef CA_MOM_PER
#define CA_MOM_PER 1
#endif
#ifndef CA_MOM_NRED
#define CA_MOM_NRED 21
#endif
constexpr int CA_PM_GPB = 32;
constexpr int CA_PM_NO = (CA_PL_R + 1) * 16;
constexpr int CA_PM_MAXW = 8;

struct ca_pm_lds {
  double pw[CA_PM_GPB][CA_PL_R + 1];
  double Mg[CA_PM_GPB][16];
  int binof[CA_PM_GPB];
  unsigned int present[(CA_PL_NB + 31) / 32];
  float smn[CA_PM_MAXW], smx[CA_PM_MAXW], sxm[CA_PM_MAXW];
  int gave_up;
};

struct ca_pm_args {
  const float* V; unsigned int* xbits; const float* muA; const float* muB; const float* Lb; int G, C;
  ca_poly_hdr* hdr; double* part; unsigned int* bad_word; double* mirror; double seq;
// ... 87 lines not shown
      __syncthreads();
    }
    const int g0 = (grp0 + gi) * GPB;
    if (t < GPB) {
      const int g = g0 + t;
      if (g < G) {
        const double v = (double)V[g];
        int b = (int)floor((v - vlo) / delta);
        b = b < 0 ? 0 : (b >= nb ? nb - 1 : b);
        s.binof[t] = b;
        atomicOr(&s.present[b >> 5], 1u << (b & 31));
        const double dv = v - (vlo + ((double)b + 0.5) * delta);
        double p = 1.0;
#pragma unroll
        for (int k = 0; k <= R; ++k) { s.pw[t][k] = p; p = p * dv * (1.0 / (double)(k + 1)); }
        const double ma = (double)a.muA[g], mb = (double)a.muB[g];
        for (int c = 0; c < 8; ++c) {
          const double l = c < C ? (double)a.Lb[(int64_t)g * CA_CW + c] : 0.0;
          s.Mg[t][c] = ma * l; s.Mg[t][8 + c] = mb * l;
        }
      } else s.binof[t] = -1;
    }
    __syncthreads();
    const int ng = min(GPB, G - g0);
    double* mine = a.part + (int64_t)(grp0 + gi) * NB * NO;
    for (int o = t; o < NO; o += TB) {
      const int k = o >> 4, col = o & 15;
      double a0 = 0.0, a1 = 0.0, a2 = 0.0, a3 = 0.0;
      if (nb == 1) {
#pragma unroll 8
        for (int i = 0; i < ng; ++i) a0 += s.pw[i][k] * s.Mg[i][col];
      } else {
#pragma unroll 4
        for (int i = 0; i < ng; ++i) {
          const double pr = s.pw[i][k] * s.Mg[i][col];
          const int bi = s.binof[i];
          a0 += bi == 0 ? pr : 0.0; a1 += bi == 1 ? pr : 0.0; a2 += bi == 2 ? pr : 0.0; a3 += bi == 3 ? pr : 0.0;
        }
      }
      ca_pm_st<PUB>(mine + 0 * NO + o, a0);
      if (nb > 1) ca_pm_st<PUB>(mine + 1 * NO + o, a1);
      if (nb > 2) ca_pm_st<PUB>(mine + 2 * NO + o, a2);
      if (nb > 3) ca_pm_st<PUB>(mine + 3 * NO + o, a3);
      for (int b = 4; b < nb; ++b) {
        double acc = 0.0;
        if ((s.present[b >> 5] >> (b & 31)) & 1u)
          for (int i = 0; i < ng; ++i) acc += s.binof[i] == b ? s.pw[i][k] * s.Mg[i][col] : 0.0;
        ca_pm_st<PUB>(mine + (int64_t)b * NO + o, acc);
      }
    }
  }
}

template <bool DEV>
__device__ __forceinline__ void ca_pm_red_body(const double* __restrict__ part, int nblk, int64_t stride, int nout, int mode, int C, double* __restrict__ out,
                                               int wave0, int nwave) {
  const int lane = threadIdx.x & 63;
  auto ld = [&](const double* p) -> double {
    if (DEV) return __longlong_as_double((long long)__hip_atomic_load(reinterpret_cast<const unsigned long long*>(p), __ATOMIC_RELAXED, __HIP_MEMORY_SCOPE_AGENT));
    return *p;
  };
  for (int j = wave0; j < nout; j += nwave) {
    double v[8];
#pragma unroll
    for (int u = 0; u < 8; ++u) { const int blk = lane + 64 * u; v[u] = blk < nblk ? ld(part + (int64_t)blk * stride + j) : 0.0; }
    double a = 0.0;
#pragma unroll
    for (int u = 0; u < 8; ++u) a += v[u];
    for (int blk = lane + 512; blk < nblk; blk += 64) a += ld(part + (int64_t)blk * stride + j);
#pragma unroll
    for (int o = 32; o > 0; o >>= 1) a += __shfl_xor(a, o, 64);
    if (lane == 0) {
      if (mode == 1) {
        const int k = (j / C) % (CA_PL_R + 2);
        double f = 1.0;
        for (int i = 2; i <= k; ++i) f *= (double)i;
        a /= f;
      }
      out[j] = a;
    }
  }
}

template <int TB>
__device__ __forceinline__ void ca_pm_ride_block(const ca_pm_args& a, int blk, unsigned char* lds) {
  ca_pm_lds& s = *reinterpret_cast<ca_pm_lds*>(lds);
  const int t = threadIdx.x;
  if (blk < a.nmb) {
    const int grp0 = blk * a.per;
    ca_pm_B_body<TB, true>(a, grp0, min(a.per, a.ngrp - grp0), blk == 0, s);
    asm volatile("s_waitcnt vmcnt(0)" ::: "memory");
    __syncthreads();
    if (t == 0) __hip_atomic_store(a.flags + blk, a.tag, __ATOMIC_RELAXED, __HIP_MEMORY_SCOPE_AGENT);
    return;
  }
  if (t == 0) s.gave_up = 0;
  __syncthreads();
  {
    const unsigned long long t0 = __builtin_amdgcn_s_memrealtime();
    for (int i = t; i < a.nmb; i += TB) {
      while (__hip_atomic_load(a.flags + i, __ATOMIC_RELAXED, __HIP_MEMORY_SCOPE_AGENT) != a.tag) {
        if (__builtin_amdgcn_s_memrealtime() - t0 > a.timeout_ticks) {
          __hip_atomic_store(a.err, 1u, __ATOMIC_RELAXED, __HIP_MEMORY_SCOPE_SYSTEM);
          s.gave_up = 1;
          break;
        }
        __builtin_amdgcn_s_sleep(2);
      }
    }
  }
  __builtin_amdgcn_fence(__ATOMIC_ACQUIRE, "agent");
  __syncthreads();
  if (s.gave_up) return;
  const int r = blk - a.nmb;
  if (r == 0 && t == 0) *a.xbits = 0u;
  const int nb = __hip_atomic_load(&a.hdr->nb, __ATOMIC_RELAXED, __HIP_MEMORY_SCOPE_AGENT);
  ca_pm_red_body<true>(a.part, a.ngrp, (int64_t)CA_PL_NB * CA_PM_NO, nb * CA_PM_NO, 0, a.C, a.tabB, r * (TB / 64) + (t >> 6), a.nred * (TB / 64));
}
```

clonealign_amd/csrc/clonealign_hip.hip:

```cpp
#include "clonealign_hip.h"

#include <dlfcn.h>
#include <unistd.h>
#include <hip/hip_runtime.h>

#include <algorithm>
#include <cmath>
#include <cstdio>
#include <cstring>
#include <string>
#include <atomic>
#include <chrono>
#include <thread>
#include <vector>

#include "ca_kernels.hip.h"
#include "ca_poly.h"
#include "philox_host.h"

#include "ca_eng_state.inc"
#include "ca_eng_launch.inc"
#include "ca_eng_reduce.inc"
#include "ca_eng_loop.inc"
#include "ca_eng_ingest.inc"
// ... 23 lines not shown
    for (int c = 0; c < C; ++c) mx = std::max(mx, L[hidx(layout, g, c, G, C)]);
    if (mx > pp.max_copy_number) kg[g] = 0;
  }
  for (int g = 0; g < G; ++g) if (kg[g] && !(col[g] > pp.min_counts_per_gene)) kg[g] = 0;
  if (pp.remove_outlying_genes) {
    std::vector<double> gm;
    for (int g = 0; g < G; ++g) if (kg[g]) gm.push_back(col[g] / (double)N);
    if (!gm.empty()) {
      auto median = [](std::vector<double> v) {
        std::sort(v.begin(), v.end());
        const size_t n = v.size();
        return n % 2 ? v[n / 2] : 0.5 * (v[n / 2 - 1] + v[n / 2]);
      };
      const double med = median(gm);
      std::vector<double> dev(gm.size());
      for (size_t i = 0; i < gm.size(); ++i) dev[i] = std::fabs(gm[i] - med);
      const double md = 1.4826 * median(dev);
      double mean = 0.0;
      for (double v : gm) mean += v;
      mean /= (double)gm.size();
      const double thr = mean + pp.nmads * md;
      for (int g = 0; g < G; ++g) if (kg[g] && col[g] / (double)N > thr) kg[g] = 0;
    }
  }
  if (pp.remove_genes_same_copy_number && C >= 2) {
    for (int g = 0; g < G; ++g) {
      if (!kg[g]) continue;
      double m = 0.0;
      for (int c = 0; c < C; ++c) m += L[hidx(layout, g, c, G, C)];
      m /= C;
      double v = 0.0;
      for (int c = 0; c < C; ++c) { const double d = L[hidx(layout, g, c, G, C)] - m; v += d * d; }
      if (v / (C - 1) == 0.0) kg[g] = 0;
    }
  }
  PCK2(hipMemcpy(dkeep, kg.data(), (size_t)G, hipMemcpyHostToDevice));
  if (layout == CA_COL_MAJOR)
    hipLaunchKernelGGL((k_pre_rowsum_cm<ST>), dim3(cdiv(N, CA_TB)), dim3(CA_TB), 0, 0, src, dkeep, N, G, sn, sg, drow);
  else
    hipLaunchKernelGGL((k_pre_rowsum<ST>), dim3(cdiv(N, CA_TB / 64)), dim3(CA_TB), 0, 0, src, dkeep, N, G, sn, sg, drow);
  PCK2(hipGetLastError());
  std::vector<double> row((size_t)N);
  PCK2(hipMemcpy(row.data(), drow, (size_t)N * sizeof(double), hipMemcpyDeviceToHost));
  for (int64_t n = 0; n < N; ++n) keep_cell[n] = row[n] > pp.min_counts_per_cell ? 1 : 0;
  memcpy(keep_gene, kg.data(), (size_t)G);
  if (gene_sums) memcpy(gene_sums, col.data(), (size_t)G * sizeof(double));
  if (cell_sums) memcpy(cell_sums, row.data(), (size_t)N * sizeof(double));
#undef PCK2
  cleanup();
  return CA_OK;
}

struct gate_snapshot {
  bool look_valid, bwd_ready, pre_valid, em_stale, y_defer, ys_quant_ready, ycache_valid, yfin_pending, fold_now;
  int64_t pre_A, pre_B, hint_A, hint_B, gaux_slot;
  int vmm_at_idx, gaux_idx, ys_steps, ys_namax[3];
  float b1p, b2p; uint64_t adam_steps;
  int poly_xglob_steps;
  float *vchi, *vchi_alt, *alpha_u, *alpha_u_alt;
  void take(const ca_engine* h) {
    look_valid = h->look_valid; bwd_ready = h->bwd_ready; pre_valid = h->pre_valid; em_stale = h->em_stale; y_defer = h->y_defer;
    ys_quant_ready = h->ys_quant_ready; ycache_valid = h->ycache_valid; yfin_pending = h->yfin_pending; fold_now = h->fold_now;
    pre_A = h->pre_A; pre_B = h->pre_B; hint_A = h->hint_A; hint_B = h->hint_B; gaux_slot = h->gaux_slot;
    vmm_at_idx = h->vmm_at_idx; gaux_idx = h->gaux_idx; ys_steps = h->ys_steps;
    for (int i = 0; i < 3; ++i) ys_namax[i] = h->ys_namax[i];
    b1p = h->b1p; b2p = h->b2p; adam_steps = h->adam_steps;
    poly_xglob_steps = h->poly_xglob_steps;
    vchi = h->vchi; vchi_alt = h->vchi_alt; alpha_u = h->alpha_u; alpha_u_alt = h->alpha_u_alt;
  }
  void restore(ca_engine* h) const {
    h->look_valid = look_valid; h->bwd_ready = bwd_ready; h->pre_valid = pre_valid; h->em_stale = em_stale; h->y_defer = y_defer;
    h->ys_quant_ready = ys_quant_ready; h->ycache_valid = ycache_valid; h->yfin_pending = yfin_pending; h->fold_now = fold_now;
    h->pre_A = pre_A; h->pre_B = pre_B; h->hint_A = -1; h->hint_B = -1; h->gaux_slot = gaux_slot;
    h->vmm_at_idx = vmm_at_idx; h->gaux_idx = gaux_idx; h->ys_steps = ys_steps;
    for (int i = 0; i < 3; ++i) h->ys_namax[i] = ys_namax[i];
    h->b1p = b1p; h->b2p = b2p; h->adam_steps = adam_steps;
    h->poly_xmax_ready = false;
    h->poly_xglob_steps = poly_xglob_steps;
    h->vchi = vchi; h->vchi_alt = vchi_alt; h->alpha_u = alpha_u; h->alpha_u_alt = alpha_u_alt;
  }
};
struct fwd_snapshot {
  double *gene_part, *gene_part_alt, *gene_partB, *gene_partB_alt;
  bool pre_valid, em_stale, yfin_pending, ys_quant_ready, ycache_valid, look_valid, bwd_ready;
  int ys_slot, ys_steps;
  int64_t look_slot;
  unsigned long long host_seq, host_seq_next;
  ca_small_args mon_tail;
  void take(const ca_engine* h) {
    gene_part = h->gene_part; gene_part_alt = h->gene_part_alt; gene_partB = h->gene_partB; gene_partB_alt = h->gene_partB_alt;
    pre_valid = h->pre_valid; em_stale = h->em_stale; yfin_pending = h->yfin_pending; ys_quant_ready = h->ys_quant_ready; ycache_valid = h->ycache_valid;
    look_valid = h->look_valid; bwd_ready = h->bwd_ready; ys_slot = h->ys_slot; ys_steps = h->ys_steps; look_slot = h->look_slot;
    host_seq = h->host_seq; host_seq_next = h->host_seq_next; mon_tail = h->mon_tail;
  }
  void restore(ca_engine* h) const {
    h->gene_part = gene_part; h->gene_part_alt = gene_part_alt; h->gene_partB = gene_partB; h->gene_partB_alt = gene_partB_alt;
    h->pre_valid = pre_valid; h->em_stale = em_stale; h->yfin_pending = yfin_pending; h->ys_quant_ready = ys_quant_ready; h->ycache_valid = ycache_valid;
    h->look_valid = look_valid; h->bwd_ready = bwd_ready; h->ys_slot = ys_slot; h->ys_steps = ys_steps; h->look_slot = look_slot;
    h->host_seq = host_seq; h->host_seq_next = host_seq_next; h->mon_tail = mon_tail;
  }
};
inline bool fwd_is_one_launch(const ca_engine* h, int64_t slotA, int64_t slotB) {
  return h->fused_ok && !h->s2 && h->fwd_cell && h->ride_ys && !h->ycache_valid && !h->y_defer && !h->y_pending && h->pre_valid && h->pre_A == slotA &&
         h->pre_B == slotB && h->ys_quant_ready && h->yfin_split && h->em_stale && h->D > 0 && h->tail_fuse && !is_sharded(h) && h->gate_local;
}
inline void gate_answer(ca_engine* h, int go) {
  volatile unsigned long long* w = reinterpret_cast<volatile unsigned long long*>(h->host_pinned + 48);
  std::atomic_thread_fence(std::memory_order_release);
  *w = (h->gate_seq << 1) | (unsigned long long)(go ? 1 : 0);
  std::atomic_thread_fence(std::memory_order_seq_cst);
}
int gate_resolve(ca_engine* h, int go) {
  gate_answer(h, go);
  if (!go) return 0;
  const double patience_us = (double)h->gate_ticks / h->ticks_per_us;
  const double us = std::chrono::duration<double, std::micro>(std::chrono::steady_clock::now() - h->gate_t0).count();
  if (patience_us >= 200.0 && us < 0.5 * patience_us) return 1;
  volatile unsigned long long* ack = reinterpret_cast<volatile unsigned long long*>(h->host_pinned + 56);
  unsigned spins = 0;
  auto t_next = std::chrono::steady_clock::now() + std::chrono::milliseconds(20);
  for (;;) {
    const unsigned long long a = *ack;
    if ((a >> 2) == h->gate_seq) return (a & 3ull) == 1ull ? 1 : 0;
    if ((++spins & 0x3FFu) == 0 && std::chrono::steady_clock::now() >= t_next) {
      t_next = std::chrono::steady_clock::now() + std::chrono::milliseconds(20);
      const hipError_t q = hipStreamQuery(h->stream);
      if (q == hipSuccess) {
        const unsigned long long a2 = *ack;
        if ((a2 >> 2) == h->gate_seq) return (a2 & 3ull) == 1ull ? 1 : 0;
        h->err = "ca_run: the gated update completed without leaving its verdict";
        return -CA_ERR_STATE;
      }
      if (q != hipErrorNotReady) { h->err = std::string("hipStreamQuery: ") + hipGetErrorString(q); return -CA_ERR_HIP; }
    }
  }
}
int gate_close(ca_engine* h) {
  if (!h->gate_open) return CA_OK;
  h->gate_open = false; h->gate_aborted = true;
  gate_answer(h, 0);
  HIPCK(h, hipStreamSynchronize(h->stream));
  if (h->gate_fsnap) h->gate_fsnap->restore(h);
  if (h->gate_snap) h->gate_snap->restore(h);
  return CA_OK;
}
#define CA_NOT_IN_RUN(h)                                                                                                                  \
  do {                                                                                                                                    \
    if ((h) && (h)->in_run) {                                                                                                             \
      (h)->err = "this call changes the engine's state and cannot be made from a ca_run_ex poll hook (read-only calls can: ca_get_param, " \
                 "ca_get_gradient, ca_get_info, ca_synchronize, ca_get_kernel_times)";                                                   \
// ... 98 lines not shown
  if (h->stream) hipStreamSynchronize(h->stream);
  if (h->stream2) { hipStreamSynchronize(h->stream2); hipStreamDestroy(h->stream2); }
  if (h->ev_params) hipEventDestroy(h->ev_params);
  if (h->ev_ydone) hipEventDestroy(h->ev_ydone);
  if (h->stream3) { hipStreamSynchronize(h->stream3); hipStreamDestroy(h->stream3); }
  if (h->ev_poly0) hipEventDestroy(h->ev_poly0);
  if (h->ev_poly1) hipEventDestroy(h->ev_poly1);
  if (h->ev_ywdone) hipEventDestroy(h->ev_ywdone);
  if (h->ev_stage) hipEventDestroy(h->ev_stage);
  if (h->comm) g_rccl.CommDestroy(h->comm);
  if (h->p2p) {
    for (void* q : h->p2p->opened) if (q) hipIpcCloseMemHandle(q);
    if (h->p2p->err_host) hipHostFree(h->p2p->err_host);
    if (h->p2p->err_local) hipFree(h->p2p->err_local);
    if (h->p2p->slab) hipFree(h->p2p->slab);
    if (h->p2p->peers_dev) hipFree(h->p2p->peers_dev);
    delete h->p2p;
  }
  for (auto& e : h->ev_pool) { hipEventDestroy(e.a); hipEventDestroy(e.b); }
  for (void* q : h->allocs) hipFree(q);
  if (h->eps_dev) hipFree(h->eps_dev);
  if (h->elbo_dev) hipFree(h->elbo_dev);
  if (h->host_pinned) hipHostFree(h->host_pinned);
  if (h->eps_stage) hipHostFree(h->eps_stage);
  if (h->host_ar_buf) hipHostFree(h->host_ar_buf);
  if (h->poly_ring) hipHostFree(h->poly_ring);
  if (h->stream) hipStreamDestroy(h->stream);
  delete h;
  return CA_OK;
}

int ca_get_info(ca_handle h, ca_info* i) {
  if (!h || !i) return CA_ERR_INVALID;
  memset(i, 0, sizeof(*i));
  i->N = h->N; i->G = h->G; i->C = h->C; i->K = h->K; i->P = h->P; i->S = h->S;
  i->y_storage = h->ystore; i->y_bytes_per_elem = h->ybytes; i->y_device_bytes = h->y_dev_bytes; i->device_bytes = h->dev_bytes;
  i->gsplit = h->gsplit; i->csplit = h->csplit; i->n_cu = h->n_cu; i->fused_sweep = h->fused_ok ? 1 : 0;
  i->fwd_mfma = ((h->fused_ok && h->fwd_mfma) || h->pfwd) ? 1 : 0; i->bwd_mfma = h->bwd_mfma ? 1 : 0; i->fsplit = h->fsplit; i->fwd_cell = (h->fused_ok && h->fwd_cell) ? 1 : 0;
  i->y_mfma = h->y_ys ? 2 : 0;
  i->y_stream_bits = h->y_ys ? (h->ys4 ? 4 : 8) : 0;
  i->y_stream_n2 = h->ys_n2;
  i->y_stream_esc = h->ys_n2 > 0 ? h->n_esc2 : h->ys4 ? h->n_esc : 0;
  i->y_stream_bytes = !h->y_ys ? 0 : h->ys_n2 > 0 ? (h->ys_N64 / 64) * (int64_t)h->ys_nseg * (h->ys_n2 * 1024 + (8 - h->ys_n2) * 2048) + 4 * h->n_esc2
                                   : h->ys4 ? h->ys_N64 * h->Gp / 2 + 4 * h->n_esc : h->ys_N64 * h->Gp;
  i->y_ride = (h->ride_ok || h->ride_ys) ? 1 : 0;
  i->transport = (h->p2p && h->p2p->connected) ? CA_TRANSPORT_P2P : h->comm ? CA_TRANSPORT_RCCL : h->host_ar ? CA_TRANSPORT_HOST : CA_TRANSPORT_NONE;
  i->red_n = h->red_n;
  i->fwd_block_cells = (h->fused_ok && h->fwd_cell) ? 16 * h->fc_tl : 0; i->fwd_blocks_big = h->fc_nbig;
  i->fwd_balanced = h->fwd_bal ? h->bal_q : 0;
  i->fwd_series = h->poly ? 1 : 0; i->series_passes = h->n_series; i->series_fallbacks = h->n_series_fallback;
  i->mom_ride = h->mom_ride ? 1 : 0;
  i->cell_lean = h->cell_lean ? 1 : 0; i->cell_mfma = h->cell_mfma ? 1 : 0;
  i->mom_last = h->mom_last ? 1 : 0; i->mom_free_slots = h->mom_free_slots;
  i->fold_gsum = (h->fold_gsum && !is_sharded(h)) ? 1 : 0; i->yfin_split = (h->yfin_split && !is_sharded(h)) ? 1 : 0;
  i->update_merge = (h->upd_merge && h->fused_ok && h->fwd_cell && h->K > 0) ? 1 : 0;
  return CA_OK;
}

int ca_stream_busy(ca_handle h, int32_t* busy) {
  if (!h || !busy) return CA_ERR_INVALID;
  const hipError_t q = hipStreamQuery(h->stream);
  if (q != hipSuccess && q != hipErrorNotReady) HIPCK(h, q);
  *busy = q == hipErrorNotReady ? 1 : 0;
  if (q == hipErrorNotReady) (void)hipGetLastError();
  return CA_OK;
}

int ca_synchronize(ca_handle h) {
  if (!h) return CA_ERR_INVALID;
  HIPCK(h, hipSetDevice(h->device));
  CACK(gate_close(h));
  SYNC(h);
  return CA_OK;
}

#include "ca_eng_comm.inc"
static int stage_one(ca_handle h, const float* eps) { return stage_eps(h, eps, 1, 1); }

int ca_gamma_init(ca_handle h, const float* eps) {
  if (!h) return CA_ERR_INVALID;
  CA_NOT_IN_RUN(h);
  HIPCK(h, hipSetDevice(h->device));
  CACK(stage_one(h, eps));
  CACK(run_pass(h, 0, CA_MODE_GINIT, 0, nullptr));
  SYNC(h);
  return CA_OK;
}

int ca_elbo(ca_handle h, const float* eps, double* elbo) {
  if (!h || !elbo) return CA_ERR_INVALID;
  CA_NOT_IN_RUN(h);
  HIPCK(h, hipSetDevice(h->device));
  CACK(stage_one(h, eps));
  CACK(run_pass(h, 0, CA_MODE_ELBO, 0, h->elbo_dev));
  return read_doubles(h, h->elbo_dev, elbo, 1);
}

int ca_elbo_terms(ca_handle h, const float* eps, double terms[3]) {
  if (!h || !terms) return CA_ERR_INVALID;
  CA_NOT_IN_RUN(h);
  HIPCK(h, hipSetDevice(h->device));
  CACK(stage_one(h, eps));
  CACK(run_pass(h, 0, CA_MODE_ELBO, 0, h->elbo_dev));
  return read_doubles(h, h->terms_dev, terms, 3);
}

// ... 242 lines not shown
int ca_ystream_parts(ca_handle h, int64_t dims[6], float* yw_part, float* yt_part, int32_t exps[2], int32_t* w_fix, int32_t* p_fix) {
  if (!h || !dims) return CA_ERR_INVALID;
  if (!h->y_ys || h->K != 1) { h->err = "ca_ystream_parts: this engine does not run the one-copy count-matrix stream"; return CA_ERR_INVALID; }
  if (!h->ys_launched) { h->err = "ca_ystream_parts: no launch of the count-matrix stream yet (ca_elbo / ca_gradients / a loop call makes one)"; return CA_ERR_STATE; }
  HIPCK(h, hipSetDevice(h->device));
  CACK(gate_close(h));
  CACK(wait_y(h, true));
  const int64_t N = h->N, Gp = h->Gp, N64 = h->ys_N64;
  dims[0] = h->ys_nseg; dims[1] = N; dims[2] = h->ys_nrg; dims[3] = Gp; dims[4] = h->ys_RS;
  dims[5] = (h->ycache_valid && !h->ys_quant_ready) ? 1 : 0;
  if (yw_part) HIPCK(h, hipMemcpyAsync(yw_part, h->YWpart, (size_t)(h->ys_nseg * N) * sizeof(float), hipMemcpyDeviceToHost, h->stream));
  if (yt_part) HIPCK(h, hipMemcpyAsync(yt_part, h->YTpart, (size_t)(h->ys_nrg * Gp) * sizeof(float), hipMemcpyDeviceToHost, h->stream));
  if (exps) HIPCK(h, hipMemcpyAsync(exps, h->ys_exps + 2 * ((h->ys_slot + 2) % 3), 2 * sizeof(int32_t), hipMemcpyDeviceToHost, h->stream));
  std::vector<signed char> wi(w_fix ? (size_t)Gp * 16 : 0), pi(p_fix ? (size_t)N64 * 16 : 0);
  if (w_fix) HIPCK(h, hipMemcpyAsync(wi.data(), h->Wr, wi.size(), hipMemcpyDeviceToHost, h->stream));
  if (p_fix) HIPCK(h, hipMemcpyAsync(pi.data(), h->Pr, pi.size(), hipMemcpyDeviceToHost, h->stream));
  SYNC(h);
  auto fix = [](const std::vector<signed char>& img, int64_t n, int32_t* out) {
    for (int64_t i = 0; i < n; ++i) {
      const signed char* d = img.data() + ((i >> 6) * 64 + 16 * ((i >> 4) & 3)) * 16 + (i & 15);
      out[i] = (int32_t)((int64_t)d[0] + (int64_t)d[16] * 256 + (int64_t)d[32] * 65536 + (int64_t)d[48] * 16777216);
    }
  };
  if (w_fix) fix(wi, Gp, w_fix);
  if (p_fix) fix(pi, N64, p_fix);
  return CA_OK;
}

int ca_set_param(ca_handle h, const char* name, const double* in) {
  if (!h || !name || !in) return CA_ERR_INVALID;
  CA_NOT_IN_RUN(h);
  HIPCK(h, hipSetDevice(h->device));
  ParamRef r;
  if (!find_param(h, name, false, r) || r.xform != 0 || r.d) { h->err = std::string("cannot set parameter: ") + name; return CA_ERR_INVALID; }
  if (r.rows * r.cols == 0) return CA_OK;
  std::vector<float> buf;
  CACK(download_f(h, buf, r.f, r.rows * std::max<int64_t>(r.stride, 1)));
  for (int64_t i = 0; i < r.rows; ++i)
    for (int64_t c = 0; c < r.cols; ++c)
      buf[i * r.stride + r.off + c] = (float)in[r.matrix ? hidx(h->layout, i, c, r.rows, r.cols) : i];
  CACK(upload_f(h, r.f, buf));
  CACK(refresh_derived(h));
  SYNC(h);
  return CA_OK;
}

int ca_reinit(ca_handle h, const double* psi0, const double* loc0) {
  if (!h) return CA_ERR_INVALID;
  CA_NOT_IN_RUN(h);
  if (h->K > 0 && !psi0) { h->err = "psi0 is required when K > 0"; return CA_ERR_INVALID; }
  HIPCK(h, hipSetDevice(h->device));
  CACK(wait_y(h, true));
  HIPCK(h, hipStreamSynchronize(h->stream));
  if (h->host_pinned) { *reinterpret_cast<volatile unsigned int*>(h->host_pinned + 41) = 0u; *reinterpret_cast<volatile unsigned int*>(h->host_pinned + 42) = 0u; *reinterpret_cast<volatile unsigned int*>(h->host_pinned + 43) = 0u; }
  SYNC(h);
  const int64_t N = h->N; const int G = h->G, C = h->C, K = h->K, D = h->D;
  auto zero = [&](float* p, int64_t n) { return p && n > 0 ? hipMemsetAsync(p, 0, (size_t)n * sizeof(float), h->stream) : hipSuccess; };
  const int64_t GD = (int64_t)G * std::max(D, 1), NK = N * std::max(K, 1);
  HIPCK(h, zero(h->V, GD)); HIPCK(h, zero(h->m_V, GD)); HIPCK(h, zero(h->v_V, GD));
  HIPCK(h, zero(h->ls, G)); HIPCK(h, zero(h->m_ls, G)); HIPCK(h, zero(h->v_ls, G));
  HIPCK(h, zero(h->m_loc, G)); HIPCK(h, zero(h->v_loc, G));
  HIPCK(h, zero(h->vchi, std::max(K, 1))); HIPCK(h, zero(h->m_v, std::max(K, 1))); HIPCK(h, zero(h->v_v, std::max(K, 1)));
  HIPCK(h, zero(h->alpha_u, C)); HIPCK(h, zero(h->m_a, C)); HIPCK(h, zero(h->v_a, C));
  HIPCK(h, zero(h->glogit, N * C)); HIPCK(h, zero(h->m_gl, N * C)); HIPCK(h, zero(h->v_gl, N * C));
  HIPCK(h, zero(h->m_psi, NK)); HIPCK(h, zero(h->v_psi, NK));
  if (loc0) {
    std::vector<float> l0((size_t)G);
    for (int g = 0; g < G; ++g) l0[g] = (float)loc0[g];
    CACK(upload_f(h, h->loc, l0));
  } else {
    HIPCK(h, hipMemcpyAsync(h->loc, h->loc_init, (size_t)G * sizeof(float), hipMemcpyDeviceToDevice, h->stream));
  }
  if (K > 0) {
    std::vector<float> Fh;
    CACK(download_f(h, Fh, h->F, N * D));
    for (int64_t n = 0; n < N; ++n)
      for (int k = 0; k < K; ++k) Fh[(size_t)n * D + k] = (float)psi0[hidx(h->layout, n, k, N, K)];
    CACK(upload_f(h, h->F, Fh));
  }
  h->b1p = (float)h->opt.beta1;
  h->b2p = (float)h->opt.beta2;
  h->mon_tail.enabled = 0;
  h->bwd_ready = false;
  h->hint_A = h->hint_B = -1;
  CACK(refresh_derived(h));
  SYNC(h);
  return CA_OK;
}

int ca_get_kernel_times(ca_handle h, double ms[CA_KERNEL_COUNT], int64_t launches[CA_KERNEL_COUNT]) {
  if (!h) return CA_ERR_INVALID;
  HIPCK(h, hipSetDevice(h->device));
  CACK(gate_close(h));
  CACK(prof_flush(h));
  for (int i = 0; i < CA_KERNEL_COUNT; ++i) {
    if (ms) ms[i] = h->k_ms[i];
    if (launches) launches[i] = h->k_n[i];
  }
  return CA_OK;
}

int ca_reset_kernel_times(ca_handle h) {
  if (!h) return CA_ERR_INVALID;
  CA_NOT_IN_RUN(h);
  CACK(prof_flush(h));
  for (int i = 0; i < CA_KERNEL_COUNT; ++i) { h->k_ms[i] = 0; h->k_n[i] = 0; }
  return CA_OK;
// ... 89 lines not shown
```

clonealign_amd/engine.py:

```python
import ctypes as C
import os

import numpy as np

from . import hostprep

_HERE = os.path.dirname(os.path.abspath(__file__))
LIB_PATH = os.path.join(_HERE, "libclonealign_hip.so")

CA_OK = 0
CA_ERR_NAN = 4
CA_INTERRUPTED = 7
CA_ABI_VERSION = 6
P2P_HANDLE_BYTES = 128
CA_F64, CA_F32, CA_I32, CA_U16, CA_U8 = 0, 1, 2, 3, 4
CA_ROW_MAJOR, CA_COL_MAJOR = 0, 1
YSTORE = {"auto": 0, "f32": 1, "u16": 2, "u8": 3}
YSTORE_NAME = {v: k for k, v in YSTORE.items()}
KERNEL_NAMES = ("fwd", "bwd", "ypass", "cell", "other")
VARIANTS = {"fused": 1 << 0, "fwd_mfma": 1 << 1, "fwd_cell": 1 << 2, "bwd_mfma": 1 << 3, "tail_fuse": 1 << 4, "async_y": 1 << 5,
            "pre": 1 << 6, "pair_elbo": 1 << 7, "prep_fast": 1 << 8, "update_merge": 1 << 9, "p2p": 1 << 10, "fold_gsum": 1 << 11, "y_ride": 1 << 12, "ride_seq": 1 << 13, "y_mfma1": 1 << 14, "yfin_ride": 1 << 15, "p2p_ride": 1 << 16, "run_gate": 1 << 17, "s2_fuse": 1 << 18, "fwd_bal": 1 << 19, "bwd_tl3": 1 << 20, "series": 1 << 21, "y4": 1 << 22, "mom_ride": 1 << 23, "cell_lean": 1 << 24, "mom_last": 1 << 25, "cell_mfma": 1 << 26, "y2": 1 << 27}
VARIANTS_ON = {"y_mfma2": 1 << 0, "async_small": 1 << 1, "y_mfma1": 1 << 2, "fold_always": 1 << 3, "ride_seq": 1 << 4, "p2p_same_device": 1 << 5, "run_fwd": 1 << 6, "bal_tiles": 1 << 7, "series": 1 << 8, "y4": 1 << 9, "mom_last": 1 << 10, "y2": 1 << 11}
OPT_VERBOSE = 0x80000000
TUNE = {"gsplit": 0, "fsplit": 1, "fc_tl": 2, "fc_nbig": 3, "csplit": 4, "csplit_m": 5, "tr": 6, "rg": 7}
TRANSPORT_NAME = {0: "none", 1: "rccl", 2: "host", 3: "p2p"}

EXPORTS = (
    "ca_abi_version", "ca_build_id", "ca_device_count", "ca_default_options", "ca_create", "ca_destroy", "ca_last_error", "ca_get_info",
    "ca_synchronize", "ca_stream_busy", "ca_comm_unique_id", "ca_comm_init", "ca_p2p_export", "ca_p2p_connect", "ca_p2p_commit", "ca_comm_benchmark", "ca_comm_selftest", "ca_set_host_allreduce", "ca_gamma_init", "ca_elbo", "ca_elbo_terms",
    "ca_step", "ca_gradients", "ca_run", "ca_run_ex", "ca_iterate", "ca_final_elbo", "ca_init_psi_pca", "ca_clone_gene_sums", "ca_get_param", "ca_set_param",
    "ca_get_gradient", "ca_reinit", "ca_get_kernel_times", "ca_reset_kernel_times", "ca_set_profile", "ca_eps_draw", "ca_allele_loglik", "ca_preprocess",
    "ca_group_create", "ca_group_destroy", "ca_group_last_error", "ca_group_get_info", "ca_group_rank_handle", "ca_group_init_psi_pca", "ca_group_gamma_init",
    "ca_group_elbo", "ca_group_step", "ca_group_run_ex", "ca_group_iterate", "ca_group_final_elbo", "ca_group_get_param", "ca_group_reinit",
    "ca_group_clone_gene_sums",
    "ca_create_sparse", "ca_group_create_sparse",
    "ca_fit_mse", "ca_group_fit_mse",
    "ca_logexpr_sums", "ca_group_logexpr_sums",
    "ca_clone_loglik", "ca_group_clone_loglik",
    "ca_project_cells", "ca_group_project_cells",
    "ca_clone_pair_loglik", "ca_group_clone_pair_loglik",
    "ca_clone_loglik_dm", "ca_group_clone_loglik_dm",
    "ca_clone_loglik_by_block", "ca_group_clone_loglik_by_block",
    "ca_simulate_counts", "ca_simulate_kernel_ms",
    "ca_predictive_stats", "ca_predictive_kernel_ms",
    "ca_predictive_moments", "ca_predictive_moments_kernel_ms",
    "ca_clone_evidence", "ca_group_clone_evidence",
    "ca_clone_loglik_reweighted", "ca_group_clone_loglik_reweighted", "ca_reweighted_kernel_ms",
    "ca_ystream_parts",
)
CA_BOOT_RCHUNK = 32


def reweighted_cells_per_batch(n, G, C, D, R):
    rc = min(int(R), CA_BOOT_RCHUNK)
    nzc, nw = -(-int(G) // 512), -(-int(C) // 32)
    nc1, nc2 = -(-rc * (C + 1) // 16) * 16, -(-rc * C // 16) * 16
    per_cell = (nzc * (nc1 + (nc2 + 1 if D > 0 else 0)) + rc * (C + 1) + 2 * C) * 8 + (rc * nw + C) * 4
    return min(int(n), max(256, ((1 << 28) // per_cell) // 256 * 256))
CA_SPARSE_CSR, CA_SPARSE_CSC = 0, 1


class CaProblem(C.Structure):
    _fields_ = [("N", C.c_int64), ("G", C.c_int32), ("C", C.c_int32), ("K", C.c_int32), ("P", C.c_int32),
                ("S", C.c_int32), ("layout", C.c_int32), ("y_dtype", C.c_int32), ("y_on_device", C.c_int32),
                ("Y", C.c_void_p), ("L", C.c_void_p), ("psi0", C.c_void_p), ("loc0", C.c_void_p),
                ("X", C.c_void_p), ("extra_loglik", C.c_void_p),
                ("N_src", C.c_int64), ("G_src", C.c_int32), ("cell_index", C.c_void_p), ("gene_index", C.c_void_p),
                ("y_ld", C.c_int64)]


class CaSparse(C.Structure):
    _fields_ = [("kind", C.c_int32), ("val_dtype", C.c_int32), ("index_bytes", C.c_int32), ("on_device", C.c_int32),
                ("nnz", C.c_int64), ("ptr", C.c_void_p), ("idx", C.c_void_p), ("val", C.c_void_p)]


class CaOptions(C.Structure):
    _fields_ = [("learning_rate", C.c_double), ("beta1", C.c_double), ("beta2", C.c_double),
                ("adam_eps", C.c_double), ("seed", C.c_uint64), ("device", C.c_int32),
                ("y_storage", C.c_int32), ("rank", C.c_int32), ("world", C.c_int32), ("profile", C.c_int32),
                ("variant_off", C.c_uint32), ("tune", C.c_int32 * 8), ("variant_on", C.c_uint32),
                ("ride_pattern", C.c_int32), ("comm_timeout_ms", C.c_int32), ("gate_timeout_us", C.c_int32), ("reserved", C.c_int32 * 2)]


class CaInfo(C.Structure):
    _fields_ = [("N", C.c_int64), ("G", C.c_int32), ("C", C.c_int32), ("K", C.c_int32), ("P", C.c_int32),
                ("S", C.c_int32), ("y_storage", C.c_int32), ("y_bytes_per_elem", C.c_int32),
                ("y_device_bytes", C.c_int64), ("device_bytes", C.c_int64), ("gsplit", C.c_int32),
                ("csplit", C.c_int32), ("n_cu", C.c_int32), ("fused_sweep", C.c_int32), ("fwd_mfma", C.c_int32),
                ("bwd_mfma", C.c_int32), ("fsplit", C.c_int32), ("fwd_cell", C.c_int32), ("y_mfma", C.c_int32),
                ("transport", C.c_int32), ("y_ride", C.c_int32), ("red_n", C.c_int64),
                ("fwd_block_cells", C.c_int32), ("fwd_blocks_big", C.c_int32), ("fold_gsum", C.c_int32), ("yfin_split", C.c_int32),
                ("update_merge", C.c_int32), ("fwd_balanced", C.c_int32), ("fwd_series", C.c_int32), ("y_stream_bits", C.c_int32),
                ("series_passes", C.c_int64), ("series_fallbacks", C.c_int64), ("mom_ride", C.c_int32), ("cell_lean", C.c_int32),
                ("mom_last", C.c_int32), ("mom_free_slots", C.c_int32), ("cell_mfma", C.c_int32),
                ("y_stream_n2", C.c_int32), ("y_stream_esc", C.c_int64), ("y_stream_bytes", C.c_int64)]


class CaGroupInfo(C.Structure):
    _fields_ = [("world", C.c_int32), ("transport", C.c_int32), ("p2p_status", C.c_int32), ("rccl_status", C.c_int32),
                ("rebuilds", C.c_int32), ("selftest_rounds", C.c_int32), ("N", C.c_int64), ("note", C.c_char * 384)]


class CaPreprocessParams(C.Structure):
    _fields_ = [("min_counts_per_gene", C.c_double), ("min_counts_per_cell", C.c_double),
                ("remove_outlying_genes", C.c_int32), ("remove_genes_same_copy_number", C.c_int32),
                ("nmads", C.c_double), ("max_copy_number", C.c_double)]


HOST_ALLREDUCE_FN = C.CFUNCTYPE(C.c_int, C.c_void_p, C.POINTER(C.c_double), C.c_int64)
POLL_FN = C.CFUNCTYPE(C.c_int, C.c_void_p, C.c_int32, C.c_double)

_lib = None


def _ptr(a, empty_null=False):
    return None if a is None or (empty_null and a.size == 0) else a.ctypes.data_as(C.c_void_p)


def load_library(path=None):
    global _lib
    if _lib is not None and path is None:
        return _lib
    p = path or os.environ.get("CLONEALIGN_HIP_LIB") or LIB_PATH
    if not os.path.exists(p):
        raise RuntimeError(
            f"{p} not found: build the HIP engine first (python -c 'import __graft_entry__ as g; g.build()' "
            "or make -C clonealign_amd/csrc). clonealign_amd has no CPU fallback.")
    lib = C.CDLL(p)
    lib.ca_last_error.restype = C.c_char_p
    lib.ca_last_error.argtypes = [C.c_void_p]
    lib.ca_build_id.restype = C.c_char_p
    lib.ca_build_id.argtypes = []
    lib.ca_group_last_error.restype = C.c_char_p
    lib.ca_group_last_error.argtypes = [C.c_void_p]
    for name in EXPORTS:
        if name not in ("ca_last_error", "ca_build_id", "ca_group_last_error"):
            getattr(lib, name).restype = C.c_int
    lib.ca_device_count.argtypes = [C.POINTER(C.c_int32)]
    lib.ca_create.argtypes = [C.POINTER(CaProblem), C.POINTER(CaOptions), C.POINTER(C.c_void_p)]
    lib.ca_create_sparse.argtypes = [C.POINTER(CaProblem), C.POINTER(CaSparse), C.POINTER(CaOptions), C.POINTER(C.c_void_p)]
    lib.ca_destroy.argtypes = [C.c_void_p]
    lib.ca_get_info.argtypes = [C.c_void_p, C.POINTER(CaInfo)]
    lib.ca_synchronize.argtypes = [C.c_void_p]
    lib.ca_stream_busy.argtypes = [C.c_void_p, C.POINTER(C.c_int32)]
    lib.ca_ystream_parts.argtypes = [C.c_void_p, C.POINTER(C.c_int64), C.c_void_p, C.c_void_p, C.c_void_p, C.c_void_p, C.c_void_p]
    lib.ca_comm_unique_id.argtypes = [C.c_char_p]
    lib.ca_comm_init.argtypes = [C.c_void_p, C.c_char_p]
    lib.ca_p2p_export.argtypes = [C.c_void_p, C.c_char_p]
# ... 950 lines not shown
```

include/clonealign_hip.h:

```cpp
#ifndef CLONEALIGN_HIP_H
#define CLONEALIGN_HIP_H

#include <stdint.h>

#ifdef __cplusplus
extern "C" {
#endif

#define CA_ABI_VERSION 6

typedef struct ca_engine* ca_handle;

enum ca_status {
  CA_OK = 0,
  CA_ERR_INVALID = 1,
  CA_ERR_HIP = 2,
  CA_ERR_NOMEM = 3,
  CA_ERR_NAN = 4,
  CA_ERR_COMM = 5,
  CA_ERR_STATE = 6,
  CA_INTERRUPTED = 7
};

enum ca_dtype { CA_F64 = 0, CA_F32 = 1, CA_I32 = 2, CA_U16 = 3, CA_U8 = 4 };
enum ca_layout { CA_ROW_MAJOR = 0, CA_COL_MAJOR = 1 };
enum ca_ystore { CA_YSTORE_AUTO = 0, CA_YSTORE_F32 = 1, CA_YSTORE_U16 = 2, CA_YSTORE_U8 = 3 };

typedef struct ca_problem {
  int64_t N;
  int32_t G, C;
  int32_t K, P, S;
  int32_t layout;
  int32_t y_dtype;
  int32_t y_on_device;
  const void* Y;
  const double* L;
  const double* psi0;
  const double* loc0;
  const double* X;
  const double* extra_loglik;
  int64_t N_src;
  int32_t G_src;
  const int64_t* cell_index;
  const int32_t* gene_index;
  int64_t y_ld;
} ca_problem;

enum ca_variant {
  CA_VAR_FUSED = 1 << 0,
  CA_VAR_FWD_MFMA = 1 << 1,
  CA_VAR_FWD_CELL = 1 << 2,
  CA_VAR_BWD_MFMA = 1 << 3,
  CA_VAR_TAIL_FUSE = 1 << 4,
  CA_VAR_ASYNC_Y = 1 << 5,
  CA_VAR_PRE = 1 << 6,
  CA_VAR_PAIR_ELBO = 1 << 7,
  CA_VAR_PREP_FAST = 1 << 8,
  CA_VAR_UPDATE_MERGE = 1 << 9,
  CA_VAR_P2P_RIDE = 1 << 16,
  CA_VAR_RUN_GATE = 1 << 17,
  CA_VAR_S2_FUSE = 1 << 18,
  CA_VAR_FWD_BAL = 1 << 19,
  CA_VAR_BWD_TL3 = 1 << 20,
  CA_VAR_SERIES = 1 << 21,
  CA_VAR_P2P = 1 << 10,
  CA_VAR_FOLD_GSUM = 1 << 11,
  CA_VAR_Y_RIDE = 1 << 12,
  CA_VAR_Y_MFMA1 = 1 << 14,
  CA_VAR_YFIN_RIDE = 1 << 15,
  CA_VAR_Y4 = 1 << 22,
  CA_VAR_MOM_RIDE = 1 << 23,
  CA_VAR_CELL_LEAN = 1 << 24,
  CA_VAR_MOM_LAST = 1 << 25,
  CA_VAR_CELL_MFMA = 1 << 26,
  CA_VAR_Y2 = 1 << 27,
  CA_VAR_RIDE_SEQ = 1 << 13
};
enum ca_variant_on {
  CA_VARX_Y_MFMA2 = 1 << 0,
  CA_VARX_Y_MFMA1 = 1 << 2,
  CA_VARX_FOLD_ALWAYS = 1 << 3,
  CA_VARX_RIDE_SEQ = 1 << 4,
  CA_VARX_P2P_SAME_DEVICE = 1 << 5,
  CA_VARX_RUN_FWD = 1 << 6,
  CA_VARX_BAL_TILES = 1 << 7,
  CA_VARX_SERIES = 1 << 8,
  CA_VARX_Y4 = 1 << 9,
  CA_VARX_MOM_LAST = 1 << 10,
  CA_VARX_Y2 = 1 << 11,
  CA_VARX_ASYNC_SMALL = 1 << 1
};
#define CA_OPT_VERBOSE 0x80000000u
enum ca_tune_id {
  CA_TUNE_GSPLIT = 0, CA_TUNE_FSPLIT = 1, CA_TUNE_FC_TL = 2, CA_TUNE_FC_NBIG = 3, CA_TUNE_CSPLIT = 4, CA_TUNE_CSPLIT_M = 5,
  CA_TUNE_TR = 6, CA_TUNE_RG = 7, CA_TUNE_COUNT = 8
};

typedef struct ca_options {
  double learning_rate;
  double beta1, beta2, adam_eps;
  uint64_t seed;
  int32_t device;
  int32_t y_storage;
  int32_t rank, world;
  int32_t profile;
  uint32_t variant_off;
  int32_t tune[8];
  uint32_t variant_on;
  int32_t ride_pattern;
  int32_t comm_timeout_ms;
  int32_t gate_timeout_us;
  int32_t reserved[2];
} ca_options;

typedef struct ca_info {
  int64_t N;
  int32_t G, C, K, P, S;
  int32_t y_storage;
  int32_t y_bytes_per_elem;
  int64_t y_device_bytes;
  int64_t device_bytes;
  int32_t gsplit, csplit;
  int32_t n_cu;
  int32_t fused_sweep;
  int32_t fwd_mfma;
  int32_t bwd_mfma;
  int32_t fsplit;
  int32_t fwd_cell;
  int32_t y_mfma;
  int32_t transport;
  int32_t y_ride;
  int64_t red_n;
  int32_t fwd_block_cells;
  int32_t fwd_blocks_big;
  int32_t fold_gsum;
  int32_t yfin_split;
  int32_t update_merge;
  int32_t fwd_balanced;
  int32_t fwd_series;
  int32_t y_stream_bits;
  int64_t series_passes;
  int64_t series_fallbacks;
  int32_t mom_ride;
  int32_t cell_lean;
  int32_t mom_last;
  int32_t mom_free_slots;
  int32_t cell_mfma;
  int32_t y_stream_n2;
  int64_t y_stream_esc;
  int64_t y_stream_bytes;
} ca_info;
enum ca_transport { CA_TRANSPORT_NONE = 0, CA_TRANSPORT_RCCL = 1, CA_TRANSPORT_HOST = 2, CA_TRANSPORT_P2P = 3 };

enum ca_kernel_id {
  CA_KERNEL_FWD = 0,
  CA_KERNEL_BWD = 1,
  CA_KERNEL_YPASS = 2,
  CA_KERNEL_CELL = 3,
  CA_KERNEL_OTHER = 4,
  CA_KERNEL_COUNT = 5
};

int ca_abi_version(void);
const char* ca_build_id(void);
int ca_device_count(int32_t* n);
int ca_default_options(ca_options* opts);

int ca_create(const ca_problem* problem, const ca_options* opts, ca_handle* out);

enum ca_sparse_kind { CA_SPARSE_CSR = 0,
                      CA_SPARSE_CSC = 1 };
typedef struct ca_sparse {
  int32_t kind;
  int32_t val_dtype;
  int32_t index_bytes;
  int32_t on_device;
  int64_t nnz;
  const void* ptr;
  const void* idx;
  const void* val;
} ca_sparse;
int ca_create_sparse(const ca_problem* problem, const ca_sparse* y, const ca_options* opts, ca_handle* out);
int ca_destroy(ca_handle h);
const char* ca_last_error(ca_handle h);
int ca_get_info(ca_handle h, ca_info* info);
int ca_synchronize(ca_handle h);
int ca_stream_busy(ca_handle h, int32_t* busy);
int ca_ystream_parts(ca_handle h, int64_t dims[6], float* yw_part, float* yt_part, int32_t exps[2], int32_t* w_fix, int32_t* p_fix);

int ca_comm_unique_id(char id[128]);
int ca_comm_init(ca_handle h, const char id[128]);
#define CA_P2P_HANDLE_BYTES 128
int ca_p2p_export(ca_handle h, char handle[CA_P2P_HANDLE_BYTES]);
int ca_p2p_connect(ca_handle h, const char* handles );
int ca_p2p_commit(ca_handle h, int32_t all_ranks_ok);
int ca_comm_benchmark(ca_handle h, int32_t transport, int32_t n_calls, int64_t n_doubles, double* us_per_call);
int ca_comm_selftest(ca_handle h, int32_t n_rounds, int64_t n_doubles, int64_t* n_bad);
typedef int (*ca_host_allreduce_fn)(void* user, double* buf, int64_t n);
int ca_set_host_allreduce(ca_handle h, ca_host_allreduce_fn fn, void* user);

int ca_gamma_init(ca_handle h, const float* eps);
int ca_elbo(ca_handle h, const float* eps, double* elbo);
int ca_elbo_terms(ca_handle h, const float* eps, double terms[3]);
// ... 165 lines not shown
```

Baseline: 10320 iterations/s.

## Merge series-form reduction into gene backward kernel with in-kernel flag wait

Splits the series-form cell kernel from its reduction and, on a single unsharded device, defers the reduction so it runs inside a merged backward gene kernel. Gene blocks wait on reducer flags with a timeout. The change also moves the count-matrix column finish onto the reducer or merged launch when cell count is small. This is meant to cut a kernel launch and its serialization per iteration, at the cost of spin-wait synchronization inside one launch and new error paths. For 100000 cells the column move is off, but the merge path is on by default.

```diff
diff --git a/clonealign_amd/csrc/ca_eng_create.inc b/clonealign_amd/csrc/ca_eng_create.inc
--- a/clonealign_amd/csrc/ca_eng_create.inc
+++ b/clonealign_amd/csrc/ca_eng_create.inc
@@ -489,6 +489,8 @@
   }
   h->cell_lean = h->poly && variant_on(h, CA_VAR_CELL_LEAN, "CA_CELL_LEAN");
   h->cell_mfma = h->poly && variant_on(h, CA_VAR_CELL_MFMA, "CA_CELL_MFMA");
+  h->gene_ride = h->poly && variant_on(h, CA_VAR_GENE_RIDE, "CA_GENE_RIDE");
+  h->gene_cols = h->gene_ride && (h->opt.reserved[1] == 8 || (h->opt.reserved[1] != 7 && Nn <= CA_GENE_COLS_MAXN));
   h->ride_ok = h->ystore == CA_YSTORE_U8 && K == 1 && D <= 2 && h->fused_ok && !h->c16 && h->fwd_cell && (h->fc_tl == 6 || h->fc_tl == 8 || (h->fc_tl == 2 && h->fc_nbig == 0)) &&
                !h->y_ys && variant_on(h, CA_VAR_Y_RIDE, "CA_Y_RIDE");
   const bool tl1_ok = h->fc_tl == 1 && h->fc_nbig == 0 && !h->c16;
diff --git a/clonealign_amd/csrc/ca_eng_loop.inc b/clonealign_amd/csrc/ca_eng_loop.inc
--- a/clonealign_amd/csrc/ca_eng_loop.inc
+++ b/clonealign_amd/csrc/ca_eng_loop.inc
@@ -32,7 +32,7 @@
   CACK(make_etamax(h));
   h->gaux_slot = -1;
   h->ycache_valid = false;
-  h->yfin_pending = false;
+  h->yfin_pending = false; h->ycol_pending = false;
   h->look_valid = false;
   h->poly_fresh = false;
   h->poly_seq_base = h->poly_seq + 1;
@@ -60,8 +60,9 @@
   a.YWpart = h->YWpart; a.nseg = nseg + (h->n_ovf > 0 ? 1 : 0); a.F = h->F; a.D = h->D; a.N = h->N; a.YW = h->YW; a.yw_part = h->yw_part;
   return a;
 }
-int launch_yfinish(ca_engine* h, int rows, int nseg) {
-  const ca_yfin_args a = yfin_args(h, rows, nseg);
+int launch_yfinish(ca_engine* h, int rows, int nseg, bool cols_only = false) {
+  ca_yfin_args a = yfin_args(h, rows, nseg);
+  if (cols_only) a.nrow = 0;
   LAUNCH(h, CA_KERNEL_OTHER, hipLaunchKernelGGL(k_yfinish, dim3(a.ncol + a.nrow), dim3(1024), 0, h->stream, a.part, a.out, a.rows, a.ld, a.cols, a.col_chunk_ptr,
                                                 a.csum, h->K, a.G, a.ncol, a.YWpart, a.nseg, a.F, a.D, a.N, a.YW, a.yw_part));
   return CA_OK;
@@ -107,12 +108,17 @@
 }
 ca_ovf_args ys_ovf(ca_engine* h) { return ovf_args(h, h->YWpart + (int64_t)h->ys_nseg * h->N); }
 int yfin_flush(ca_engine* h) {
+  if (h->ycol_pending && !h->yfin_pending) {
+    h->ycol_pending = false;
+    return launch_yfinish(h, h->ys_nrg, h->ys_nseg, true);
+  }
+  h->ycol_pending = false;
   if (!h->yfin_pending) return CA_OK;
   h->yfin_pending = false;
   return launch_yfinish(h, h->ys_nrg, h->ys_nseg);
 }
 int ys_finish(ca_engine* h, bool defer = false) {
-  h->yfin_pending = true;
+  h->yfin_pending = true; h->ycol_pending = false;
   if (!defer) CACK(yfin_flush(h));
   h->ys_slot = (h->ys_slot + 1) % 3;
   h->ys_launched = true;
@@ -173,7 +179,7 @@
     return CA_OK;
   }
   if (h->ycache_valid || h->K == 0) { h->ycache_valid = true; return yfin_flush(h); }
-  h->yfin_pending = false;
+  h->yfin_pending = false; h->ycol_pending = false;
   if (h->y_ys) return ycache_ys(h);
   dim3 grid((unsigned)((int64_t)h->nrg * h->nseg));
   const ca_ovf_args ovf = ovf_args(h, h->YWpart + (int64_t)h->nseg * h->N * h->K);
@@ -258,6 +264,12 @@
   if (h->poly_fresh) {
     h->poly_fresh = false;
     h->fold_now = false;
+    const bool merged_back = h->red_pending && gene_ride_merges(h);
+    if (h->red_pending && !merged_back) HIPCK(h, ca_poly_reduce(h->stream, &h->pws, h->N, h->C, nullptr, nullptr, nullptr, 0, h->F, nullptr, 0, 1));
+    h->red_pending = false;
+    ca_yfin_args back_cols;
+    memset(&back_cols, 0, sizeof(back_cols));
+    if (merged_back && h->ycol_pending && !h->yfin_pending) { back_cols = yfin_args(h, h->ys_nrg, h->ys_nseg); back_cols.nrow = 0; h->ycol_pending = false; }
     CACK(yfin_flush(h));
     ca_small_args bwd_tail = no_small_args();
     if (is_sharded(h)) {
@@ -289,7 +301,12 @@
     }
     else if (h->mon_tail.enabled) { CACK(wait_y(h, false)); bwd_tail = h->mon_tail; h->mon_tail.enabled = 0; }
     CACK(prof_begin(h, CA_KERNEL_BWD));
-    const hipError_t e = ca_poly_backward(h->stream, &h->pws, h->V, mu32, h->Lb, h->G, h->C, h->red + h->off_g, &bwd_tail);
+    hipError_t e;
+    if (merged_back) {
+      if (++h->gene_tag == 0u) h->gene_tag = 1u;
+      e = ca_poly_backward_merged(h->stream, &h->pws, h->V, mu32, h->Lb, h->G, h->C, h->red + h->off_g, &bwd_tail, back_cols.ncol > 0 ? &back_cols : nullptr,
+                                  h->poly_nb_ub, h->gene_tag, 50000000ull, reinterpret_cast<unsigned int*>(h->host_dev + 44));
+    } else e = ca_poly_backward(h->stream, &h->pws, h->V, mu32, h->Lb, h->G, h->C, h->red + h->off_g, &bwd_tail);
     HIPCK(h, e);
     CACK(prof_end(h));
     h->poly_df = true;
@@ -300,6 +317,7 @@
     ca_yfin_args yfin;
     memset(&yfin, 0, sizeof(yfin));
     ride_ar = is_sharded(h) && p2p_ride_ok(h, h->red_n);
+    if (h->ycol_pending) CACK(yfin_flush(h));
     if (is_sharded(h) && !ride_ar) CACK(yfin_flush(h));
     if (h->yfin_pending) { yfin = yfin_args(h, h->ys_nrg, h->ys_nseg); h->yfin_pending = false; }
     ca_small_args bwd_tail = no_small_args();
@@ -426,7 +444,7 @@
   h->poly_xmax_ready = xmax_ready;
   if (h->poly_xglob_steps >= 0) h->poly_xglob_steps += 1;
   h->ycache_valid = false;
-  h->yfin_pending = false;
+  h->yfin_pending = false; h->ycol_pending = false;
   h->look_valid = false;
   if (h->poly && h->y_ys && h->K > 0) h->poly_y_defer = true;
 }
@@ -649,6 +667,7 @@
     steps = (int)(h->adam_steps - h->poly_steps_at[(s - CA_POLY_LAG) % 16]);
   }
   *use_series = ca_poly_covers(r[0], r[1], r[2], steps, poly_step_bound(h));
+  h->poly_nb_ub = *use_series ? ca_poly_nb_ahead(r[0], r[1], r[2], steps, poly_step_bound(h)) : 0;
   h->poly_seq = s;
   h->poly_steps_at[s % 16] = h->adam_steps;
   return CA_OK;
@@ -760,6 +779,7 @@
     if (mom_left) { h->err = "internal: the series form's moments were to ride on a count-matrix stream launch that was not made"; return CA_ERR_STATE; }
     h->ys_defer_next = false;
     ca_yfin_args yfin_ride;
+    memset(&yfin_ride, 0, sizeof(yfin_ride));
     const bool yfin_rides = h->yfin_pending;
     if (yfin_rides) { yfin_ride = yfin_args(h, h->ys_nrg, h->ys_nseg); h->yfin_pending = false; }
     if (moments_aside) HIPCK(h, hipStreamWaitEvent(h->stream, h->ev_poly1, 0));
@@ -772,9 +792,16 @@
       if (h->K > 0) { ltail.yw_part = h->yw_part; ltail.n_yw = h->n_yw; }
       ltail.reduce_only = 1; ltail.host_out = nullptr;
     }
-    e = ca_poly_cells(h->stream, &h->pws, h->N, h->C, h->K, &cp, h->alpha_u, h->cell_part, h->dFpart, yfin_rides ? &yfin_ride : nullptr,
-                      sh ? &ltail : nullptr, h->poly_xmax_ready ? h->poly_xpart : nullptr, (int)cdiv(h->N, CA_TB), h->F, sh ? h->red + h->off_x : nullptr,
-                      h->opt.rank, std::max(h->opt.world, 1), h->cell_lean, h->cell_mfma);
+    const bool cols_move = yfin_rides && h->gene_cols;
+    const bool merges = gene_ride_merges(h);
+    ca_yfin_args yfin_cols = yfin_ride;
+    if (cols_move) yfin_ride.ncol = 0;
+    e = ca_poly_cells(h->stream, &h->pws, h->N, h->C, h->K, &cp, h->alpha_u, h->cell_part, h->dFpart, yfin_rides ? &yfin_ride : nullptr, h->cell_lean, h->cell_mfma);
+    h->red_pending = merges;
+    if (merges) h->ycol_pending = cols_move;
+    else if (e == hipSuccess)
+      e = ca_poly_reduce(h->stream, &h->pws, h->N, h->C, cols_move ? &yfin_cols : nullptr, sh ? &ltail : nullptr, h->poly_xmax_ready ? h->poly_xpart : nullptr,
+                         (int)cdiv(h->N, CA_TB), h->F, sh ? h->red + h->off_x : nullptr, h->opt.rank, std::max(h->opt.world, 1));
     h->mon_tail_local = sh;
     if (sh) { h->poly_xslot_pending = true; h->poly_xglob_steps = -1; }
     HIPCK(h, e);
diff --git a/clonealign_amd/csrc/ca_eng_reduce.inc b/clonealign_amd/csrc/ca_eng_reduce.inc
--- a/clonealign_amd/csrc/ca_eng_reduce.inc
+++ b/clonealign_amd/csrc/ca_eng_reduce.inc
@@ -1,4 +1,5 @@
 inline bool is_sharded(const ca_engine* h) { return h->opt.world > 1 || h->comm || h->host_ar || (h->p2p && h->p2p->connected); }
+inline bool gene_ride_merges(const ca_engine* h) { return h->gene_ride && !is_sharded(h) && h->host_dev != nullptr; }
 struct ca_ar_ride {
   const float* gpart = nullptr; int nslice = 0; int64_t fold_lo = 0, fold_n = 0;
   const double* yw_part = nullptr; int n_yw = 0; int64_t yw_index = -1;
diff --git a/clonealign_amd/csrc/ca_eng_state.inc b/clonealign_amd/csrc/ca_eng_state.inc
--- a/clonealign_amd/csrc/ca_eng_state.inc
+++ b/clonealign_amd/csrc/ca_eng_state.inc
@@ -63,6 +63,9 @@
   for (int t = 1; t <= 200000; ++t) { p1 *= b1; p2 *= b2; sup = std::max(sup, std::sqrt(1.0 - p2) / (1.0 - p1)); }
   return lr * sup * (1.0 - b1) / std::sqrt((1.0 - b2) * (1.0 - b1 * b1 / b2));
 }
+#ifndef CA_GENE_COLS_MAXN
+#define CA_GENE_COLS_MAXN 65536
+#endif
 struct ca_engine {
   int64_t N = 0;
   int G = 0, C = 0, K = 0, P = 0, S = 0, D = 0;
@@ -139,6 +142,8 @@
   bool mom_last = false, mom_ovf_first = false; int mom_free_slots = 0, mom_per = CA_MOM_PER, mom_nred = CA_MOM_NRED;
   bool cell_mfma = false;
   bool cell_lean = false;
+  bool gene_cols = false;
+  bool gene_ride = false, red_pending = false, ycol_pending = false; unsigned gene_tag = 0; int poly_nb_ub = 0;
   bool poly = false, poly_side = false, poly_y_defer = false, poly_fresh = false, poly_df = false ; ca_poly_ws pws; float* poly_zero = nullptr; unsigned char* poly_mem = nullptr;
   float *Mb2 = nullptr, *mu32B = nullptr, *Zpart2 = nullptr; double* gene_partB = nullptr;
   bool y_defer = false;
@@ -215,6 +220,10 @@
     h->err = "a reducer block of the series form's moment role gave up waiting for the moment blocks of its launch (k_ys_mfma_mom); the engine's state is undefined";
     return CA_ERR_STATE;
   }
+  if (h->host_pinned && *reinterpret_cast<volatile unsigned int*>(h->host_pinned + 44) != 0u) {
+    h->err = "a gene block of the series form's merged way back gave up waiting for the reducer blocks of its launch (k_poly_tail); the engine's state is undefined";
+    return CA_ERR_STATE;
+  }
   if (h->host_pinned && *reinterpret_cast<volatile unsigned int*>(h->host_pinned + 42) != 0u) {
     h->err = "the series form of the contraction (CA_VARX_SERIES) cannot cover this fit's exponent range: max|psi| (max W - min W) exceeds 4 x " +
              std::to_string(CA_PL_NB) + " bins' worth; the passes since are truncated -- start over without the series form";
diff --git a/clonealign_amd/csrc/ca_poly.h b/clonealign_amd/csrc/ca_poly.h
--- a/clonealign_amd/csrc/ca_poly.h
+++ b/clonealign_amd/csrc/ca_poly.h
@@ -11,8 +11,9 @@
 #endif
 
 struct ca_poly_hdr { double vlo, delta, xmax; int nb, bad; };
+#define CA_PL_NGFLAG 256
 struct ca_poly_ws {
-  ca_poly_hdr* hdr; unsigned int* xbits; unsigned int* mflags ; double *tabB, *partB, *tabQ, *Qpart;
+  ca_poly_hdr* hdr; unsigned int* xbits; unsigned int* mflags ; unsigned int* gflags ; double *tabB, *partB, *tabQ, *Qpart;
   int n_cell_blocks, n_gene_blocks;
 };
 
@@ -26,16 +27,33 @@
 hipError_t ca_poly_ranges(hipStream_t st, const ca_poly_ws* w, const float* V, const float* F, int G, int64_t N, double* mirror, double seq, const float* xpart, int nx,
                           const double* xglob, int nglob, double xadd);
 hipError_t ca_poly_xslot(hipStream_t st, const float* xpart, int nx, const float* F, int64_t N, double* slots, int rank, int world);
+inline double ca_poly_bins_ahead(double xmax, double vlo, double vhi, int steps, double step_bound) {
+  const double x = xmax + steps * step_bound, wdt = (vhi - vlo) + 2.0 * steps * step_bound;
+  return x * wdt / (2.0 * CA_PL_A);
+}
 inline bool ca_poly_covers(double xmax, double vlo, double vhi, int steps, double step_bound) {
-  const double x = xmax + steps * step_bound, wdt = (vhi - vlo) + 2.0 * steps * step_bound;
-  return x == x && wdt == wdt && x * wdt <= 2.0 * CA_PL_A * CA_PL_NB;
+  const double b = ca_poly_bins_ahead(xmax, vlo, vhi, steps, step_bound);
+  return b == b && b <= (double)CA_PL_NB;
+}
+inline int ca_poly_nb_ahead(double xmax, double vlo, double vhi, int steps, double step_bound) {
+  const double b = ca_poly_bins_ahead(xmax, vlo, vhi, steps, step_bound);
+  if (!(b == b) || b > (double)CA_PL_NB) return 0;
+  const int nb = (int)b + ((double)(int)b < b ? 1 : 0);
+  return nb < 1 ? 1 : nb;
 }
 hipError_t ca_poly_cells(hipStream_t st, const ca_poly_ws* w, int64_t N, int C, int K, const void* cell_ptrs, const float* alpha_u, double* cell_part, float* dF,
                          const void* yfin_args ,
-                         const void* local_tail ,
-                         const float* xs_part, int xs_n, const float* xs_F, double* xs_slots ,
-                         int rank, int world,
                          bool lean ,
                          bool mfma );
+hipError_t ca_poly_reduce(hipStream_t st, const ca_poly_ws* w, int64_t N, int C,
+                          const void* yfin_cols ,
+                          const void* local_tail ,
+                          const float* xs_part, int xs_n, const float* xs_F, double* xs_slots ,
+                          int rank, int world);
 hipError_t ca_poly_backward(hipStream_t st, const ca_poly_ws* w, const float* V, const float* mu, const float* Lb, int G, int C, double* red_g,
                             const void* small_tail );
+hipError_t ca_poly_backward_merged(hipStream_t st, const ca_poly_ws* w, const float* V, const float* mu, const float* Lb, int G, int C, double* red_g,
+                                   const void* small_tail, const void* yfin_cols ,
+                                   int nb_hint ,
+                                   unsigned int tag , unsigned long long timeout_ticks ,
+                                   unsigned int* err );
diff --git a/clonealign_amd/csrc/ca_poly.hip b/clonealign_amd/csrc/ca_poly.hip
--- a/clonealign_amd/csrc/ca_poly.hip
+++ b/clonealign_amd/csrc/ca_poly.hip
@@ -297,66 +297,37 @@
   __syncthreads();
   if ((int)threadIdx.x < a.world) a.slots[threadIdx.x] = (int)threadIdx.x == a.rank ? (double)fmaxf(fmaxf(sx[0], sx[1]), fmaxf(sx[2], sx[3])) : 0.0;
 }
+template <bool COLS>
 __global__ void __launch_bounds__(CA_TB) k_poly_red(const double* __restrict__ part, int nblk, int64_t stride, const ca_poly_hdr* __restrict__ hdr, int per_bin,
                                                     int mode, int C, double* __restrict__ out, unsigned int* __restrict__ xbits, int nred, ca_small_args tail,
-                                                    ca_xslot_args xs) {
+                                                    ca_xslot_args xs, int nfix, ca_yfin_args yfin) {
   if ((int)blockIdx.x >= nred) {
     const int e = (int)blockIdx.x - nred;
-    if (e == 0 && tail.enabled) ca_final_small_body(tail);
+    if (COLS && e >= nfix) {
+      if constexpr (COLS) {
+        const int job = (e - nfix) * (CA_TB / 64) + (int)(threadIdx.x >> 6);
+        if (job < yfin.ncol) ca_yfin_col_wave(yfin, job);
+      }
+    }
+    else if (e == 0 && tail.enabled) ca_final_small_body(tail);
     else if (xs.slots) ca_poly_xslot_body(xs);
     return;
   }
   if (xbits && blockIdx.x == 0 && threadIdx.x == 0) *xbits = 0u;
   ca_pm_red_body<false>(part, nblk, stride, hdr->nb * per_bin, mode, C, out, blockIdx.x * (CA_TB / 64) + (threadIdx.x >> 6), nred * (CA_TB / 64));
 }
+
+#include "ca_polygene.hip.h"
 
 __global__ void __launch_bounds__(CA_TB) k_poly_gene(const ca_poly_hdr* __restrict__ hdr, const double* __restrict__ tabQ, const float* __restrict__ V,
                                                      const float* __restrict__ mu, const float* __restrict__ Lb, int G, int C,
                                                      double* __restrict__ red_g , ca_small_args tail, int ngblk) {
-  constexpr int RQ = R + 2;
   if ((int)blockIdx.x >= ngblk) {
     if (tail.enabled) ca_final_small_body(tail);
     return;
   }
-  constexpr int NBL = CA_PL_NBL;
-  __shared__ double s_tq[NBL][RQ * 8];
-  const int nb = hdr->nb;
-  const double vlo = hdr->vlo, delta = hdr->delta;
-  for (int i = threadIdx.x; i < (nb < NBL ? nb : NBL) * RQ * C; i += CA_TB) s_tq[i / (RQ * C)][i % (RQ * C)] = tabQ[i];
-  __syncthreads();
-  const int g = blockIdx.x * CA_TB + threadIdx.x;
-  if (g >= G) return;
-  const double v = (double)V[g];
-  int b = (int)floor((v - vlo) / delta);
-  b = b < 0 ? 0 : (b >= nb ? nb - 1 : b);
-  const double dv = v - (vlo + ((double)b + 0.5) * delta);
-  float lrow[8];
-  {
-    const float4 l0 = *reinterpret_cast<const float4*>(Lb + (int64_t)g * CA_CW), l1 = *reinterpret_cast<const float4*>(Lb + (int64_t)g * CA_CW + 4);
-    lrow[0] = l0.x; lrow[1] = l0.y; lrow[2] = l0.z; lrow[3] = l0.w; lrow[4] = l1.x; lrow[5] = l1.y; lrow[6] = l1.z; lrow[7] = l1.w;
-  }
-  double s0 = 0.0, s1 = 0.0;
-#define CA_PL_GENE(TQ)                                                            \
-  _Pragma("unroll")                                                               \
-  for (int c = 0; c < 8; ++c) {                                                   \
-    if (c < C) {                                                                  \
-      double tn = (TQ)[(R + 1) * C + c], tk = (TQ)[R * C + c];                    \
-      double q = tk, dq = (double)(R + 1) * tn;                                   \
-      _Pragma("unroll 10")                                                        \
-      for (int k = R - 1; k >= 0; --k) {                                          \
-        tn = tk; tk = (TQ)[k * C + c];                                            \
-        q = q * dv + tk;                                                          \
-        dq = dq * dv + (double)(k + 1) * tn;                                      \
-      }                                                                           \
-      const double l = (double)lrow[c];                                           \
-      s0 += l * q; s1 += l * dq;                                                  \
-    }                                                                             \
-  }
-  if (nb <= NBL) { CA_PL_GENE(s_tq[b]) }
-  else { const double* tq = tabQ + (int64_t)b * RQ * C; CA_PL_GENE(tq) }
-#undef CA_PL_GENE
-  red_g[(int64_t)g * 2 + 0] = s0;
-  red_g[(int64_t)g * 2 + 1] = (double)mu[g] * s1;
+  __shared__ double s_tq[CA_PL_NBL][(R + 2) * 8];
+  ca_pg_gene_block<false>(hdr, tabQ, V, mu, Lb, G, C, red_g, (int)blockIdx.x, s_tq, nullptr, nullptr);
 }
 
 inline int cdiv_i(int64_t a, int64_t b) { return (int)((a + b - 1) / b); }
@@ -366,7 +337,7 @@
 
 size_t ca_poly_workspace_bytes(int G, int n_cell_blocks) {
   const size_t nbg = (size_t)cdiv_i(G, GPB);
-  return sizeof(ca_poly_hdr) + 64 + ((nbg * sizeof(unsigned int) + 63) / 64) * 64 + sizeof(double) * ((size_t)NB * (R + 1) * 16 * (nbg + 1) + (size_t)NB * (R + 2) * 8 * ((size_t)n_cell_blocks + 1));
+  return sizeof(ca_poly_hdr) + 64 + ((nbg * sizeof(unsigned int) + 63) / 64) * 64 + CA_PL_NGFLAG * sizeof(unsigned int) + sizeof(double) * ((size_t)NB * (R + 1) * 16 * (nbg + 1) + (size_t)NB * (R + 2) * 8 * ((size_t)n_cell_blocks + 1));
 }
 
 void ca_poly_bind(ca_poly_ws* w, void* base, int G, int n_cell_blocks) {
@@ -375,6 +346,7 @@
   w->xbits = reinterpret_cast<unsigned int*>(q); q += 64;
   const size_t nbg = (size_t)cdiv_i(G, GPB);
   w->mflags = reinterpret_cast<unsigned int*>(q); q += ((nbg * sizeof(unsigned int) + 63) / 64) * 64;
+  w->gflags = reinterpret_cast<unsigned int*>(q); q += CA_PL_NGFLAG * sizeof(unsigned int);
   w->tabB = reinterpret_cast<double*>(q); q += sizeof(double) * (size_t)NB * (R + 1) * 16;
   w->partB = reinterpret_cast<double*>(q); q += sizeof(double) * (size_t)NB * (R + 1) * 16 * nbg;
   w->tabQ = reinterpret_cast<double*>(q); q += sizeof(double) * (size_t)NB * (R + 2) * 8;
@@ -414,14 +386,15 @@
   {
     ca_small_args no_tail; memset(&no_tail, 0, sizeof(no_tail));
     ca_xslot_args no_xs; memset(&no_xs, 0, sizeof(no_xs));
-    hipLaunchKernelGGL(k_poly_red, dim3(256), dim3(CA_TB), 0, st, w->partB, w->n_gene_blocks, (int64_t)NB * (R + 1) * 16, w->hdr,
-                       (R + 1) * 16, 0, C, w->tabB, w->xbits, 256, no_tail, no_xs);
+    ca_yfin_args no_yfin; memset(&no_yfin, 0, sizeof(no_yfin));
+    hipLaunchKernelGGL(k_poly_red<false>, dim3(256), dim3(CA_TB), 0, st, w->partB, w->n_gene_blocks, (int64_t)NB * (R + 1) * 16, w->hdr,
+                       (R + 1) * 16, 0, C, w->tabB, w->xbits, 256, no_tail, no_xs, 0, no_yfin);
   }
   return hipGetLastError();
 }
 
 hipError_t ca_poly_cells(hipStream_t st, const ca_poly_ws* w, int64_t N, int C, int K, const void* cell_ptrs, const float* alpha_u, double* cell_part, float* dF,
-                         const void* yfin_args, const void* local_tail, const float* xs_part, int xs_n, const float* xs_F, double* xs_slots, int rank, int world, bool lean, bool mfma) {
+                         const void* yfin_args, bool lean, bool mfma) {
   const ca_cell_ptrs& p = *static_cast<const ca_cell_ptrs*>(cell_ptrs);
   ca_yfin_args yfin;
   if (yfin_args) memcpy(&yfin, yfin_args, sizeof(yfin)); else memset(&yfin, 0, sizeof(yfin));
@@ -440,14 +413,26 @@
   }
 #undef CA_PCELL
 #undef CA_PCELL_
-  {
-    ca_small_args tail;
-    if (local_tail) memcpy(&tail, local_tail, sizeof(tail)); else memset(&tail, 0, sizeof(tail));
-    const ca_xslot_args xs = {xs_part, xs_part ? xs_n : 0, xs_F, N, xs_slots, rank, world};
-    const int nextra = (tail.enabled || xs_slots) ? 2 : 0;
-    hipLaunchKernelGGL(k_poly_red, dim3(256 + nextra), dim3(CA_TB), 0, st, w->Qpart, w->n_cell_blocks, (int64_t)NB * (R + 2) * 8, w->hdr,
-                       (R + 2) * C, 1, C, w->tabQ, nullptr, 256, tail, xs);
-  }
+  return hipGetLastError();
+}
+
+constexpr int NRED_Q = 256;
+
+hipError_t ca_poly_reduce(hipStream_t st, const ca_poly_ws* w, int64_t N, int C, const void* yfin_cols, const void* local_tail, const float* xs_part, int xs_n,
+                          const float* xs_F, double* xs_slots, int rank, int world) {
+  ca_small_args tail;
+  if (local_tail) memcpy(&tail, local_tail, sizeof(tail)); else memset(&tail, 0, sizeof(tail));
+  ca_yfin_args yfin;
+  if (yfin_cols) memcpy(&yfin, yfin_cols, sizeof(yfin)); else memset(&yfin, 0, sizeof(yfin));
+  yfin.nrow = 0;
+  const ca_xslot_args xs = {xs_part, xs_part ? xs_n : 0, xs_F, N, xs_slots, rank, world};
+  const int nfix = (tail.enabled || xs_slots) ? 2 : 0;
+  if (yfin.ncol > 0)
+    hipLaunchKernelGGL(k_poly_red<true>, dim3(NRED_Q + nfix + cdiv_i(yfin.ncol, CA_TB / 64)), dim3(CA_TB), 0, st, w->Qpart, w->n_cell_blocks, (int64_t)NB * (R + 2) * 8,
+                       w->hdr, (R + 2) * C, 1, C, w->tabQ, nullptr, NRED_Q, tail, xs, nfix, yfin);
+  else
+    hipLaunchKernelGGL(k_poly_red<false>, dim3(NRED_Q + nfix), dim3(CA_TB), 0, st, w->Qpart, w->n_cell_blocks, (int64_t)NB * (R + 2) * 8, w->hdr,
+                       (R + 2) * C, 1, C, w->tabQ, nullptr, NRED_Q, tail, xs, nfix, yfin);
   return hipGetLastError();
 }
 
@@ -460,6 +445,25 @@
   return hipGetLastError();
 }
 
+hipError_t ca_poly_backward_merged(hipStream_t st, const ca_poly_ws* w, const float* V, const float* mu, const float* Lb, int G, int C, double* red_g,
+                                   const void* small_tail, const void* yfin_cols, int nb_hint, unsigned int tag, unsigned long long timeout_ticks, unsigned int* err) {
+  if (tag == 0u || !err) return hipErrorInvalidValue;
+  ca_small_args tail;
+  if (small_tail) memcpy(&tail, small_tail, sizeof(tail)); else memset(&tail, 0, sizeof(tail));
+  ca_yfin_args yfin;
+  if (yfin_cols) memcpy(&yfin, yfin_cols, sizeof(yfin)); else memset(&yfin, 0, sizeof(yfin));
+  yfin.nrow = 0;
+  ca_gr_args a;
+  memset(&a, 0, sizeof(a));
+  a.part = w->Qpart; a.nblk = w->n_cell_blocks; a.stride = (int64_t)NB * (R + 2) * 8; a.tabQ = w->tabQ;
+  a.nred = nb_hint > 0 ? std::min(NRED_Q, std::max(1, cdiv_i((int64_t)nb_hint * (R + 2) * C, CA_TB / 64))) : NRED_Q;
+  a.hdr = w->hdr; a.V = V; a.mu = mu; a.Lb = Lb; a.G = G; a.C = C; a.red_g = red_g; a.ngblk = cdiv_i(G, CA_TB);
+  a.flags = w->gflags; a.tag = tag; a.timeout_ticks = timeout_ticks; a.err = err;
+  static_assert(NRED_Q <= CA_PL_NGFLAG, "a flag word per reducer block");
+  hipLaunchKernelGGL(k_poly_tail, dim3(a.nred + a.ngblk + (tail.enabled ? 1 : 0) + cdiv_i(yfin.ncol, CA_TB / 64)), dim3(CA_TB), 0, st, a, tail, yfin);
+  return hipGetLastError();
+}
+
 #ifdef CA_LAB
 extern "C" int ca_lab_read_cell_stamps(unsigned long long* out, int n_words) {
   return hipMemcpyFromSymbol(out, HIP_SYMBOL(ca_series::ca_lab_stamps4), (size_t)n_words * sizeof(unsigned long long)) == hipSuccess ? 0 : 2;
diff --git a/clonealign_amd/csrc/ca_polygene.hip.h b/clonealign_amd/csrc/ca_polygene.hip.h
--- /dev/null
+++ b/clonealign_amd/csrc/ca_polygene.hip.h
@@ -0,0 +1,122 @@
+#pragma once
+#include "ca_poly.h"
+
+struct ca_gr_args {
+  const double* part; int nblk; int64_t stride; double* tabQ; int nred;
+  const ca_poly_hdr* hdr; const float* V; const float* mu; const float* Lb; int G, C; double* red_g; int ngblk;
+  unsigned int* flags;
+  unsigned int tag;
+  unsigned long long timeout_ticks;
+  unsigned int* err;
+};
+
+struct ca_pg_dev_tab {
+  const double* p;
+  __device__ __forceinline__ double operator[](int i) const {
+    return __longlong_as_double((long long)__hip_atomic_load(reinterpret_cast<const unsigned long long*>(p + i), __ATOMIC_RELAXED, __HIP_MEMORY_SCOPE_AGENT));
+  }
+};
+
+template <bool RIDE>
+__device__ __forceinline__ void ca_pg_gene_block(const ca_poly_hdr* __restrict__ hdr, const double* __restrict__ tabQ, const float* __restrict__ V,
+                                                 const float* __restrict__ mu, const float* __restrict__ Lb, int G, int C, double* __restrict__ red_g, int gblk,
+                                                 double (*s_tq)[(CA_PL_R + 2) * 8], [[maybe_unused]] const ca_gr_args* ride, [[maybe_unused]] int* s_gave_up) {
+  constexpr int R = CA_PL_R, RQ = R + 2, NBL = CA_PL_NBL;
+  const int t = threadIdx.x;
+  const int nb = hdr->nb;
+  const double vlo = hdr->vlo, delta = hdr->delta;
+  if constexpr (!RIDE) {
+    for (int i = t; i < (nb < NBL ? nb : NBL) * RQ * C; i += CA_TB) s_tq[i / (RQ * C)][i % (RQ * C)] = tabQ[i];
+    __syncthreads();
+  }
+  const int g = gblk * CA_TB + t;
+  const bool live = g < G;
+  if constexpr (!RIDE) { if (!live) return; }
+  const int gg = live ? g : G - 1;
+  const double v = (double)V[gg];
+  int b = (int)floor((v - vlo) / delta);
+  b = b < 0 ? 0 : (b >= nb ? nb - 1 : b);
+  const double dv = v - (vlo + ((double)b + 0.5) * delta);
+  float lrow[8];
+  {
+    const float4 l0 = *reinterpret_cast<const float4*>(Lb + (int64_t)gg * CA_CW), l1 = *reinterpret_cast<const float4*>(Lb + (int64_t)gg * CA_CW + 4);
+    lrow[0] = l0.x; lrow[1] = l0.y; lrow[2] = l0.z; lrow[3] = l0.w; lrow[4] = l1.x; lrow[5] = l1.y; lrow[6] = l1.z; lrow[7] = l1.w;
+  }
+  [[maybe_unused]] float mug = 0.f;
+  if constexpr (RIDE) {
+    mug = mu[gg];
+    const int nout = nb * RQ * C, nw = CA_TB / 64;
+    const int need = min(ride->nred, (nout + nw - 1) / nw);
+    if (t == 0) *s_gave_up = 0;
+    __syncthreads();
+    {
+      const unsigned long long t0 = __builtin_amdgcn_s_memrealtime();
+      for (int i = t; i < need; i += CA_TB) {
+        while (__hip_atomic_load(ride->flags + i, __ATOMIC_RELAXED, __HIP_MEMORY_SCOPE_AGENT) != ride->tag) {
+          if (__builtin_amdgcn_s_memrealtime() - t0 > ride->timeout_ticks) {
+            __hip_atomic_store(ride->err, 1u, __ATOMIC_RELAXED, __HIP_MEMORY_SCOPE_SYSTEM);
+            *s_gave_up = 1;
+            break;
+          }
+          __builtin_amdgcn_s_sleep(2);
+        }
+      }
+    }
+    __builtin_amdgcn_fence(__ATOMIC_ACQUIRE, "agent");
+    __syncthreads();
+    if (*s_gave_up) return;
+    const ca_pg_dev_tab tq = {tabQ};
+    for (int i = t; i < (nb < NBL ? nb : NBL) * RQ * C; i += CA_TB) s_tq[i / (RQ * C)][i % (RQ * C)] = tq[i];
+    __syncthreads();
+    if (!live) return;
+  }
+  double s0 = 0.0, s1 = 0.0;
+#define CA_PL_GENE(TQ)                                                            \
+  _Pragma("unroll")                                                               \
+  for (int c = 0; c < 8; ++c) {                                                   \
+    if (c < C) {                                                                  \
+      double tn = (TQ)[(R + 1) * C + c], tk = (TQ)[R * C + c];                    \
+      double q = tk, dq = (double)(R + 1) * tn;                                   \
+      _Pragma("unroll 10")                                                        \
+      for (int k = R - 1; k >= 0; --k) {                                          \
+        tn = tk; tk = (TQ)[k * C + c];                                            \
+        q = q * dv + tk;                                                          \
+        dq = dq * dv + (double)(k + 1) * tn;                                      \
+      }                                                                           \
+      const double l = (double)lrow[c];                                           \
+      s0 += l * q; s1 += l * dq;                                                  \
+    }                                                                             \
+  }
+  if (nb <= NBL) { CA_PL_GENE(s_tq[b]) }
+  else if constexpr (RIDE) { const ca_pg_dev_tab tq = {tabQ + (int64_t)b * RQ * C}; CA_PL_GENE(tq) }
+  else { const double* tq = tabQ + (int64_t)b * RQ * C; CA_PL_GENE(tq) }
+#undef CA_PL_GENE
+  red_g[(int64_t)g * 2 + 0] = s0;
+  if constexpr (RIDE) red_g[(int64_t)g * 2 + 1] = (double)mug * s1;
+  else red_g[(int64_t)g * 2 + 1] = (double)mu[g] * s1;
+}
+
+__global__ void __launch_bounds__(CA_TB) k_poly_tail(ca_gr_args a, ca_small_args tail, ca_yfin_args yfin) {
+  const int blk = (int)blockIdx.x, t = threadIdx.x;
+  if (blk < a.nred) {
+    constexpr int nw = CA_TB / 64;
+    const int nout = a.hdr->nb * (CA_PL_R + 2) * a.C;
+    if (blk * nw >= nout) return;
+    ca_pm_red_body<false, true>(a.part, a.nblk, a.stride, nout, 1, a.C, a.tabQ, blk * nw + (t >> 6), a.nred * nw);
+    asm volatile("s_waitcnt vmcnt(0)" ::: "memory");
+    __syncthreads();
+    if (t == 0) __hip_atomic_store(a.flags + blk, a.tag, __ATOMIC_RELAXED, __HIP_MEMORY_SCOPE_AGENT);
+    return;
+  }
+  const int e = blk - a.nred;
+  if (e < a.ngblk) {
+    __shared__ double s_tq[CA_PL_NBL][(CA_PL_R + 2) * 8];
+    __shared__ int s_gave_up;
+    ca_pg_gene_block<true>(a.hdr, a.tabQ, a.V, a.mu, a.Lb, a.G, a.C, a.red_g, e, s_tq, &a, &s_gave_up);
+    return;
+  }
+  const int x = e - a.ngblk, ntail = tail.enabled ? 1 : 0;
+  if (x < ntail) { ca_final_small_body(tail); return; }
+  const int job = (x - ntail) * (CA_TB / 64) + (t >> 6);
+  if (job < yfin.ncol) ca_yfin_col_wave(yfin, job);
+}
diff --git a/clonealign_amd/csrc/ca_polymom.hip.h b/clonealign_amd/csrc/ca_polymom.hip.h
--- a/clonealign_amd/csrc/ca_polymom.hip.h
+++ b/clonealign_amd/csrc/ca_polymom.hip.h
@@ -163,7 +163,7 @@
   }
 }
 
-template <bool DEV>
+template <bool DEV, bool PUB = false>
 __device__ __forceinline__ void ca_pm_red_body(const double* __restrict__ part, int nblk, int64_t stride, int nout, int mode, int C, double* __restrict__ out,
                                                int wave0, int nwave) {
   const int lane = threadIdx.x & 63;
@@ -188,7 +188,7 @@
         for (int i = 2; i <= k; ++i) f *= (double)i;
         a /= f;
       }
-      out[j] = a;
+      ca_pm_st<PUB>(out + j, a);
     }
   }
 }
diff --git a/clonealign_amd/csrc/clonealign_hip.hip b/clonealign_amd/csrc/clonealign_hip.hip
--- a/clonealign_amd/csrc/clonealign_hip.hip
+++ b/clonealign_amd/csrc/clonealign_hip.hip
@@ -99,7 +99,7 @@
 }
 
 struct gate_snapshot {
-  bool look_valid, bwd_ready, pre_valid, em_stale, y_defer, ys_quant_ready, ycache_valid, yfin_pending, fold_now;
+  bool look_valid, bwd_ready, pre_valid, em_stale, y_defer, ys_quant_ready, ycache_valid, yfin_pending, ycol_pending, fold_now;
   int64_t pre_A, pre_B, hint_A, hint_B, gaux_slot;
   int vmm_at_idx, gaux_idx, ys_steps, ys_namax[3];
   float b1p, b2p; uint64_t adam_steps;
@@ -107,7 +107,7 @@
   float *vchi, *vchi_alt, *alpha_u, *alpha_u_alt;
   void take(const ca_engine* h) {
     look_valid = h->look_valid; bwd_ready = h->bwd_ready; pre_valid = h->pre_valid; em_stale = h->em_stale; y_defer = h->y_defer;
-    ys_quant_ready = h->ys_quant_ready; ycache_valid = h->ycache_valid; yfin_pending = h->yfin_pending; fold_now = h->fold_now;
+    ys_quant_ready = h->ys_quant_ready; ycache_valid = h->ycache_valid; yfin_pending = h->yfin_pending; ycol_pending = h->ycol_pending; fold_now = h->fold_now;
     pre_A = h->pre_A; pre_B = h->pre_B; hint_A = h->hint_A; hint_B = h->hint_B; gaux_slot = h->gaux_slot;
     vmm_at_idx = h->vmm_at_idx; gaux_idx = h->gaux_idx; ys_steps = h->ys_steps;
     for (int i = 0; i < 3; ++i) ys_namax[i] = h->ys_namax[i];
@@ -117,7 +117,7 @@
   }
   void restore(ca_engine* h) const {
     h->look_valid = look_valid; h->bwd_ready = bwd_ready; h->pre_valid = pre_valid; h->em_stale = em_stale; h->y_defer = y_defer;
-    h->ys_quant_ready = ys_quant_ready; h->ycache_valid = ycache_valid; h->yfin_pending = yfin_pending; h->fold_now = fold_now;
+    h->ys_quant_ready = ys_quant_ready; h->ycache_valid = ycache_valid; h->yfin_pending = yfin_pending; h->ycol_pending = ycol_pending; h->fold_now = fold_now;
     h->pre_A = pre_A; h->pre_B = pre_B; h->hint_A = -1; h->hint_B = -1; h->gaux_slot = gaux_slot;
     h->vmm_at_idx = vmm_at_idx; h->gaux_idx = gaux_idx; h->ys_steps = ys_steps;
     for (int i = 0; i < 3; ++i) h->ys_namax[i] = ys_namax[i];
@@ -129,20 +129,20 @@
 };
 struct fwd_snapshot {
   double *gene_part, *gene_part_alt, *gene_partB, *gene_partB_alt;
-  bool pre_valid, em_stale, yfin_pending, ys_quant_ready, ycache_valid, look_valid, bwd_ready;
+  bool pre_valid, em_stale, yfin_pending, ycol_pending, ys_quant_ready, ycache_valid, look_valid, bwd_ready;
   int ys_slot, ys_steps;
   int64_t look_slot;
   unsigned long long host_seq, host_seq_next;
   ca_small_args mon_tail;
   void take(const ca_engine* h) {
     gene_part = h->gene_part; gene_part_alt = h->gene_part_alt; gene_partB = h->gene_partB; gene_partB_alt = h->gene_partB_alt;
-    pre_valid = h->pre_valid; em_stale = h->em_stale; yfin_pending = h->yfin_pending; ys_quant_ready = h->ys_quant_ready; ycache_valid = h->ycache_valid;
+    pre_valid = h->pre_valid; em_stale = h->em_stale; yfin_pending = h->yfin_pending; ycol_pending = h->ycol_pending; ys_quant_ready = h->ys_quant_ready; ycache_valid = h->ycache_valid;
     look_valid = h->look_valid; bwd_ready = h->bwd_ready; ys_slot = h->ys_slot; ys_steps = h->ys_steps; look_slot = h->look_slot;
     host_seq = h->host_seq; host_seq_next = h->host_seq_next; mon_tail = h->mon_tail;
   }
   void restore(ca_engine* h) const {
     h->gene_part = gene_part; h->gene_part_alt = gene_part_alt; h->gene_partB = gene_partB; h->gene_partB_alt = gene_partB_alt;
-    h->pre_valid = pre_valid; h->em_stale = em_stale; h->yfin_pending = yfin_pending; h->ys_quant_ready = ys_quant_ready; h->ycache_valid = ycache_valid;
+    h->pre_valid = pre_valid; h->em_stale = em_stale; h->yfin_pending = yfin_pending; h->ycol_pending = ycol_pending; h->ys_quant_ready = ys_quant_ready; h->ycache_valid = ycache_valid;
     h->look_valid = look_valid; h->bwd_ready = bwd_ready; h->ys_slot = ys_slot; h->ys_steps = ys_steps; h->look_slot = look_slot;
     h->host_seq = host_seq; h->host_seq_next = host_seq_next; h->mon_tail = mon_tail;
   }
@@ -347,6 +347,7 @@
   i->mom_ride = h->mom_ride ? 1 : 0;
   i->cell_lean = h->cell_lean ? 1 : 0; i->cell_mfma = h->cell_mfma ? 1 : 0;
   i->mom_last = h->mom_last ? 1 : 0; i->mom_free_slots = h->mom_free_slots;
+  i->gene_ride = gene_ride_merges(h) ? 1 : 0;
   i->fold_gsum = (h->fold_gsum && !is_sharded(h)) ? 1 : 0; i->yfin_split = (h->yfin_split && !is_sharded(h)) ? 1 : 0;
   i->update_merge = (h->upd_merge && h->fused_ok && h->fwd_cell && h->K > 0) ? 1 : 0;
   return CA_OK;
@@ -695,7 +696,7 @@
   HIPCK(h, hipSetDevice(h->device));
   CACK(wait_y(h, true));
   HIPCK(h, hipStreamSynchronize(h->stream));
-  if (h->host_pinned) { *reinterpret_cast<volatile unsigned int*>(h->host_pinned + 41) = 0u; *reinterpret_cast<volatile unsigned int*>(h->host_pinned + 42) = 0u; *reinterpret_cast<volatile unsigned int*>(h->host_pinned + 43) = 0u; }
+  if (h->host_pinned) { *reinterpret_cast<volatile unsigned int*>(h->host_pinned + 41) = 0u; *reinterpret_cast<volatile unsigned int*>(h->host_pinned + 42) = 0u; *reinterpret_cast<volatile unsigned int*>(h->host_pinned + 43) = 0u; *reinterpret_cast<volatile unsigned int*>(h->host_pinned + 44) = 0u; }
   SYNC(h);
   const int64_t N = h->N; const int G = h->G, C = h->C, K = h->K, D = h->D;
   auto zero = [&](float* p, int64_t n) { return p && n > 0 ? hipMemsetAsync(p, 0, (size_t)n * sizeof(float), h->stream) : hipSuccess; };
diff --git a/clonealign_amd/engine.py b/clonealign_amd/engine.py
--- a/clonealign_amd/engine.py
+++ b/clonealign_amd/engine.py
@@ -19,7 +19,7 @@
 YSTORE_NAME = {v: k for k, v in YSTORE.items()}
 KERNEL_NAMES = ("fwd", "bwd", "ypass", "cell", "other")
 VARIANTS = {"fused": 1 << 0, "fwd_mfma": 1 << 1, "fwd_cell": 1 << 2, "bwd_mfma": 1 << 3, "tail_fuse": 1 << 4, "async_y": 1 << 5,
-            "pre": 1 << 6, "pair_elbo": 1 << 7, "prep_fast": 1 << 8, "update_merge": 1 << 9, "p2p": 1 << 10, "fold_gsum": 1 << 11, "y_ride": 1 << 12, "ride_seq": 1 << 13, "y_mfma1": 1 << 14, "yfin_ride": 1 << 15, "p2p_ride": 1 << 16, "run_gate": 1 << 17, "s2_fuse": 1 << 18, "fwd_bal": 1 << 19, "bwd_tl3": 1 << 20, "series": 1 << 21, "y4": 1 << 22, "mom_ride": 1 << 23, "cell_lean": 1 << 24, "mom_last": 1 << 25, "cell_mfma": 1 << 26, "y2": 1 << 27}
+            "pre": 1 << 6, "pair_elbo": 1 << 7, "prep_fast": 1 << 8, "update_merge": 1 << 9, "p2p": 1 << 10, "fold_gsum": 1 << 11, "y_ride": 1 << 12, "ride_seq": 1 << 13, "y_mfma1": 1 << 14, "yfin_ride": 1 << 15, "p2p_ride": 1 << 16, "run_gate": 1 << 17, "s2_fuse": 1 << 18, "fwd_bal": 1 << 19, "bwd_tl3": 1 << 20, "series": 1 << 21, "y4": 1 << 22, "mom_ride": 1 << 23, "cell_lean": 1 << 24, "mom_last": 1 << 25, "cell_mfma": 1 << 26, "y2": 1 << 27, "gene_ride": 1 << 28}
 VARIANTS_ON = {"y_mfma2": 1 << 0, "async_small": 1 << 1, "y_mfma1": 1 << 2, "fold_always": 1 << 3, "ride_seq": 1 << 4, "p2p_same_device": 1 << 5, "run_fwd": 1 << 6, "bal_tiles": 1 << 7, "series": 1 << 8, "y4": 1 << 9, "mom_last": 1 << 10, "y2": 1 << 11}
 OPT_VERBOSE = 0x80000000
 TUNE = {"gsplit": 0, "fsplit": 1, "fc_tl": 2, "fc_nbig": 3, "csplit": 4, "csplit_m": 5, "tr": 6, "rg": 7}
@@ -93,7 +93,7 @@
                 ("update_merge", C.c_int32), ("fwd_balanced", C.c_int32), ("fwd_series", C.c_int32), ("y_stream_bits", C.c_int32),
                 ("series_passes", C.c_int64), ("series_fallbacks", C.c_int64), ("mom_ride", C.c_int32), ("cell_lean", C.c_int32),
                 ("mom_last", C.c_int32), ("mom_free_slots", C.c_int32), ("cell_mfma", C.c_int32),
-                ("y_stream_n2", C.c_int32), ("y_stream_esc", C.c_int64), ("y_stream_bytes", C.c_int64)]
+                ("y_stream_n2", C.c_int32), ("y_stream_esc", C.c_int64), ("y_stream_bytes", C.c_int64), ("gene_ride", C.c_int32)]
 
 
 class CaGroupInfo(C.Structure):
diff --git a/include/clonealign_hip.h b/include/clonealign_hip.h
--- a/include/clonealign_hip.h
+++ b/include/clonealign_hip.h
@@ -74,6 +74,7 @@
   CA_VAR_MOM_LAST = 1 << 25,
   CA_VAR_CELL_MFMA = 1 << 26,
   CA_VAR_Y2 = 1 << 27,
+  CA_VAR_GENE_RIDE = 1 << 28,
   CA_VAR_RIDE_SEQ = 1 << 13
 };
 enum ca_variant_on {
@@ -149,6 +150,7 @@
   int32_t y_stream_n2;
   int64_t y_stream_esc;
   int64_t y_stream_bytes;
+  int32_t gene_ride;
 } ca_info;
 enum ca_transport { CA_TRANSPORT_NONE = 0, CA_TRANSPORT_RCCL = 1, CA_TRANSPORT_HOST = 2, CA_TRANSPORT_P2P = 3 };
 
```

Measured after the change: 10500 iterations/s, median of 6. 1.02x the previous value.
